# dvalcarce/filmyou-core

Hardware: AMD Instinct MI355X
Metric: top-N recs/sec (RM2), ml25m shape (higher is better)
Workload: dtype f32 (scores and logs fp32 / v_log_f32, folded in fp64; co-rating sums 64-bit fixed point in LDS (fp64 fallback); G stored as 24-bit e7m17 floats scaled per cluster above 4096 items; ratings fp16 in the row kernel when exactly representable)

## Files before the change

### filmyou-core_amd/_native.py

```python
import ctypes as C
import os
import subprocess

_HERE = os.path.dirname(os.path.abspath(__file__))
CSRC = os.path.join(_HERE, "csrc")
LIB_DIR = os.path.join(_HERE, "lib")
LIB_PATH = os.path.join(LIB_DIR, "libfilmyou_hip.so")
INCLUDE = os.path.join(os.path.dirname(_HERE), "include", "filmyou.h")
SOURCES = ["fy_api.hip", "fy_prep.hip", "fy_rm2.hip", "fy_rm2_request.hip", "fy_rm1.hip", "fy_ratings_update.hip", "fy_itemsim.hip", "fy_itemsim_request.hip", "fy_itemcf.hip", "fy_itemcf_request.hip", "fy_itemcf_estimate.hip", "fy_eval.hip", "fy_cluster.hip", "fy_nmf.hip", "fy_refine.hip", "fy_rccl.hip", "fy_seqfile.cpp"]
HEADERS = ["fy_common.hpp", "fy_tuning.hpp", "fy_rm2_plan.hpp", "fy_rm2_tables.hpp", "fy_partition.hpp", "fy_prep.hpp", "fy_cooc.hpp", "fy_cooc_tables.hpp", "fy_rm2.hpp", "fy_rm2_kernels.hpp", "fy_rm2_launch.hpp", "fy_rm2_coop.hpp", "fy_rm2_request.hpp", "fy_rm1.hpp", "fy_ratings_update.hpp", "fy_refine.hpp", "fy_itemsim_plan.hpp", "fy_itemsim_kernels.hpp", "fy_itemsim_request.hpp", "fy_itemcf_request.hpp", "fy_eval.hpp"]
HIPCC_FLAGS = ["--offload-arch=gfx950", "-O3", "-std=c++17", "-fPIC", "-shared", "-munsafe-fp-atomics", "-Wall",
               "-Wno-unused-result", "-ldl"]

SYMBOLS = [
    "fy_abi_version", "fy_last_error", "fy_context_create", "fy_context_destroy", "fy_context_synchronize", "fy_context_reload_tuning", "fy_context_inject_alloc_failure",
    "fy_context_stream", "fy_ratings_create", "fy_ratings_destroy", "fy_ratings_nnz", "fy_ratings_drop_cache", "fy_ratings_apply", "fy_ratings_copy_out", "fy_rm2_prepare",
    "fy_rm2_partial_stats", "fy_rm2_stats_layout", "fy_rm2_set_global_stats", "fy_rm2_set_collectives", "fy_rccl_unique_id", "fy_rccl_create", "fy_rccl_collectives", "fy_rccl_counters", "fy_rccl_destroy", "fy_rccl_detach_context", "fy_rm2_score", "fy_rm2_score_users", "fy_result_request_stats", "fy_rm2_job_destroy", "fy_rm2_run",
    "fy_itemsim_build", "fy_itemsim_run", "fy_itemsim_prepare", "fy_itemsim_job_destroy", "fy_itemsim_rows", "fy_result_itemsim_request_stats", "fy_itemcf_recommend", "fy_itemcf_recommend_filtered", "fy_itemcf_recommend_prepared", "fy_result_itemcf_request_stats", "fy_itemsim_job_drop_rows", "fy_ratings_shifted", "fy_itemsim_pairs",
    "fy_simpairs_write_text", "fy_idfile_read", "fy_cluster_assign", "fy_nmf_factorize", "fy_result_size", "fy_result_key0", "fy_result_key1", "fy_result_value",
    "fy_result_aux", "fy_result_n_users", "fy_result_user_id", "fy_result_user_sum", "fy_result_n_items",
    "fy_result_item_id", "fy_result_item_coll", "fy_result_total_sum", "fy_result_free", "fy_result_stats",
    "fy_seqfile_read_int_int", "fy_seqfile_read_int_double", "fy_seqfile_read_intpair_float", "fy_seqfile_write_int_int",
    "fy_seqfile_write_int_double", "fy_seqfile_write_intpair_float", "fy_mapfile_write_int_double", "fy_buffer_free",
    "fy_submap_create", "fy_submap_n_users", "fy_submap_n_items", "fy_submap_nnz", "fy_submap_counts", "fy_submap_users",
    "fy_submap_items", "fy_submap_matrix", "fy_submap_destroy", "fy_cluster_refine", "fy_refined_n_users", "fy_refined_n_counts",
    "fy_refined_clustering", "fy_refined_layout", "fy_refined_h_size", "fy_refined_w_size", "fy_refined_factors",
    "fy_refined_stats", "fy_refined_free",
    "fy_ratings_holdout", "fy_result_create_lists", "fy_eval_prepare", "fy_eval_lists", "fy_eval_destroy",
    "fy_itemcf_estimate_prepared", "fy_itemcf_estimate_ratings", "fy_result_itemcf_estimate_stats", "fy_eval_estimates",
]


def _stale():
    if not os.path.exists(LIB_PATH):
        return True
    t = os.path.getmtime(LIB_PATH)
    deps = [os.path.join(CSRC, f) for f in SOURCES + HEADERS] + [INCLUDE]
    return any(os.path.getmtime(d) > t for d in deps)


def build(force=False, verbose=False):
    if not force and not _stale():
        build_host_driver()
        return LIB_PATH
    from concurrent.futures import ThreadPoolExecutor
    obj_dir = os.path.join(LIB_DIR, "obj")
    os.makedirs(obj_dir, exist_ok=True)
    hipcc = os.environ.get("HIPCC", "/opt/rocm/bin/hipcc")
    if not os.path.exists(hipcc):
        hipcc = "hipcc"
    cflags = [f for f in HIPCC_FLAGS if f not in ("-shared", "-ldl")]
    common = max(os.path.getmtime(d) for d in [os.path.join(CSRC, h) for h in HEADERS] + [INCLUDE])
    import hashlib
    stamp_path = os.path.join(obj_dir, "flags.stamp")
    stamp = hashlib.sha256(("\0".join([os.path.realpath(hipcc)] + cflags)).encode()).hexdigest()
    try:
        with open(stamp_path) as f:
            same_flags = f.read().strip() == stamp
    except OSError:
        same_flags = False
    if not same_flags:
        force = True

    def compile_one(src):
        path, obj = os.path.join(CSRC, src), os.path.join(obj_dir, src + ".o")
        if not force and os.path.exists(obj) and os.path.getmtime(obj) > max(common, os.path.getmtime(path)):
            return obj
        cmd = [hipcc] + cflags + ["-c", "-o", obj, path]
        if verbose:
            print(" ".join(cmd))
        subprocess.run(cmd, check=True)
        return obj

    with ThreadPoolExecutor(max_workers=min(len(SOURCES), os.cpu_count() or 1)) as ex:
        objs = list(ex.map(compile_one, SOURCES))
    with open(stamp_path, "w") as f:
        f.write(stamp + "\n")
    cmd = [hipcc, "--offload-arch=gfx950", "-fPIC", "-shared", "-o", LIB_PATH] + objs + ["-ldl"]
    if verbose:
        print(" ".join(cmd))
    subprocess.run(cmd, check=True)
    build_host_driver()
    return LIB_PATH


HOST_DIR = os.path.join(_HERE, "host")
HOST_DRIVER = os.path.join(HOST_DIR, "rm2_main")


def build_host_driver():
    src = os.path.join(HOST_DIR, "rm2_main.cpp")
    hdr = os.path.join(HOST_DIR, "filmyou_job.hpp")
    if os.path.exists(HOST_DRIVER) and all(os.path.getmtime(HOST_DRIVER) >= os.path.getmtime(p) for p in (src, hdr, LIB_PATH)):
        return HOST_DRIVER
    subprocess.run(["g++", "-std=c++17", "-O2", "-Wall", "-o", HOST_DRIVER, src, "-L" + LIB_DIR, "-lfilmyou_hip",
                    "-Wl,-rpath,$ORIGIN/../lib"], check=True)
    return HOST_DRIVER


class RM2Params(C.Structure):
    _fields_ = [("lambda_", C.c_double), ("number_of_items", C.c_int32), ("number_of_recommendations", C.c_int32),
                ("filter_users", C.c_int32), ("number_of_clusters", C.c_int32), ("rank", C.c_int32),
                ("world", C.c_int32), ("flags", C.c_uint32), ("workspace_bytes", C.c_int64)]


ALL_GATHER_FN = C.CFUNCTYPE(C.c_int, C.c_void_p, C.c_void_p, C.c_void_p, C.c_int64, C.c_void_p)
REDUCE_SCATTER_FN = C.CFUNCTYPE(C.c_int, C.c_void_p, C.c_void_p, C.c_void_p, C.c_int64, C.c_void_p)


class Collectives(C.Structure):
    _fields_ = [("user", C.c_void_p), ("all_gather", ALL_GATHER_FN), ("reduce_scatter_f32", REDUCE_SCATTER_FN)]


class NMFParams(C.Structure):
    _fields_ = [("number_of_users", C.c_int32), ("number_of_items", C.c_int32), ("number_of_clusters", C.c_int32),
                ("number_of_iterations", C.c_int32), ("ppc", C.c_int32), ("normalization_frequency", C.c_int32)]


class RefineParams(C.Structure):
    _fields_ = [("number_of_users", C.c_int32), ("number_of_clusters", C.c_int32), ("users_per_sub_cluster", C.c_int32),
                ("number_of_iterations", C.c_int32), ("ppc", C.c_int32), ("normalization_frequency", C.c_int32),
                ("seed", C.c_uint64)]


class RefineStats(C.Structure):
    _fields_ = [("ms_mappings", C.c_double), ("ms_iterations", C.c_double), ("ms_assign", C.c_double), ("ms_total", C.c_double),
                ("launches", C.c_int64), ("sum_users", C.c_int64), ("sum_items", C.c_int64), ("sum_k", C.c_int64),
                ("nnz", C.c_int64), ("collisions", C.c_int64)]

    def as_dict(self):
        return {k: getattr(self, k) for k, _ in self._fields_}


class ItemSimParams(C.Structure):
    _fields_ = [("similarity", C.c_int32), ("max_similarities_per_item", C.c_int32), ("exclude_self", C.c_int32),
                ("has_threshold", C.c_int32), ("threshold", C.c_double), ("rank", C.c_int32), ("world", C.c_int32),
                ("flags", C.c_uint32), ("min_prefs_per_user", C.c_int32), ("max_prefs_per_user", C.c_int32)]


class ItemCFParams(C.Structure):
    _fields_ = [("num_recommendations", C.c_int32), ("max_prefs_per_user", C.c_int32), ("boolean_data", C.c_int32),
                ("rank", C.c_int32), ("world", C.c_int32), ("flags", C.c_uint32)]


class ItemCFFilter(C.Structure):
    _fields_ = [("has_users", C.c_int32), ("has_items", C.c_int32), ("n_users", C.c_int64), ("users", C.c_void_p),
                ("n_items", C.c_int64), ("items", C.c_void_p)]


class RM2Request(C.Structure):
    _fields_ = [("n_users", C.c_int64), ("users", C.c_void_p)]


class RM2RequestStats(C.Structure):
    _fields_ = [("users_asked", C.c_int64), ("users_known", C.c_int64), ("clusters_touched", C.c_int64), ("batches", C.c_int64),
                ("slab_rows", C.c_int64), ("slab_bytes_peak", C.c_int64), ("slab_pair_contribs", C.c_int64),
                ("full_pass_clusters", C.c_int64)]

    def as_dict(self):
        return {k: getattr(self, k) for k, _ in self._fields_}


class ItemSimRequest(C.Structure):
# ... 205 lines not shown
```

### filmyou-core_amd/csrc/fy_api.hip

```cpp
#include <algorithm>
#include <cstdlib>
#include <memory>
#include <mutex>
#include <new>
#include <unordered_map>

#include "fy_prep.hpp"
#include "fy_rm2.hpp"
#include "fy_ratings_update.hpp"
#include "fy_rm2_request.hpp"
#include "fy_itemsim_request.hpp"
#include "fy_itemcf_request.hpp"
#include "fy_eval.hpp"

namespace fy {
static thread_local char g_err[512] = "";
void set_error(const char* fmt, ...) {
    va_list ap;
    va_start(ap, fmt);
    vsnprintf(g_err, sizeof g_err, fmt, ap);
    va_end(ap);
}
const char* last_error() { return g_err; }
}

using namespace fy;

void fy::load_tuning_from_env(Tuning& t) {
    t = Tuning{};
    if (const char* e = getenv("FY_M24")) t.pack24 = atoi(e) != 0;
    if (const char* e = getenv("FY_M24_MIN_ITEMS")) t.pack24_min_items = std::max(0, atoi(e));
    if (const char* e = getenv("FY_SCORE_SLICES")) t.max_slices = atoi(e);
    if (const char* e = getenv("FY_SCORE_UPW")) { int v = atoi(e); if (v >= 1) t.users_per_wave = v; }
    if (const char* e = getenv("FY_PRUNE")) t.prune = atoi(e) != 0;
    if (const char* e = getenv("FY_LAZY_MIRROR")) t.lazy_mirror = atoi(e) != 0;
    if (const char* e = getenv("FY_REFINE")) t.refine = atoi(e) != 0;
    if (const char* e = getenv("FY_REFINE_C")) { double v = atof(e); if (v >= 0.0 && v < 1e6) t.refine_c = (float)v; }
    if (const char* e = getenv("FY_FULL_WALK_SPARSE")) t.full_walk_sparse = atoi(e) != 0;
    if (const char* e = getenv("FY_PREP_PACKED")) t.prep_packed = atoi(e) != 0;
    if (const char* e = getenv("FY_OVERLAP_VALUES")) t.overlap_values = atoi(e) != 0;
    if (const char* e = getenv("FY_SHARD_PREP")) t.shard_prep = atoi(e) != 0;
    if (const char* e = getenv("FY_SUP_BOUNDS")) t.sup_bounds = atoi(e) != 0;
    if (const char* e = getenv("FY_COOP")) t.coop = atoi(e) != 0;
    if (const char* e = getenv("FY_COOP_FORCE")) t.coop_force = atoi(e) != 0;
    if (const char* e = getenv("FY_COOC_PK")) t.cooc_pk = atoi(e) != 0;
    if (const char* e = getenv("FY_COOC_F32")) t.cooc_f32 = atoi(e) != 0;
    if (const char* e = getenv("FY_COOC_HALF")) t.cooc_half = atoi(e) != 0;
    if (const char* e = getenv("FY_COOC_RECT")) t.cooc_rect = atoi(e) != 0;
    if (const char* e = getenv("FY_COOC_FX")) t.cooc_fx = atoi(e) != 0;
    if (const char* e = getenv("FY_PANEL_MIN_CLUSTERS")) { int v = atoi(e); if (v >= 1) t.panel_min_clusters = v; }
    if (const char* e = getenv("FY_PANEL_COLS")) { int v = atoi(e); if (v >= 256) { t.panel_cols = v; t.panel_wide_below_users = 0; } }
    if (const char* e = getenv("FY_PANEL_WIDE_BELOW_USERS")) { int v = atoi(e); if (v >= 0) t.panel_wide_below_users = v; }
    if (const char* e = getenv("FY_PANEL_MAX_CH")) { int v = atoi(e); if (v >= 256) t.panel_max_ch = v; }
    if (const char* e = getenv("FY_COOC_PLANES")) t.cooc_planes = atoi(e) != 0;
    if (const char* e = getenv("FY_SCORE_HEAVY")) { int v = atoi(e); if (v >= 0) t.score_heavy = v; }
    if (const char* e = getenv("FY_SCORE_WALK")) t.score_walk = atoi(e) != 0;
    if (const char* e = getenv("FY_COOC_EPI")) t.cooc_epi = atoi(e) != 0;
    if (const char* e = getenv("FY_TOPN_SEED_XL")) t.topn_seed_xl = atoi(e) != 0;
    if (const char* e = getenv("FY_PANEL_REPAIR")) t.panel_repair = atoi(e) != 0;
    if (const char* e = getenv("FY_PANEL_MULTI_LAUNCH")) t.panel_multi_launch = atoi(e) != 0;
    if (const char* e = getenv("FY_FLAT")) t.flat_batch = atoi(e) != 0;
    if (const char* e = getenv("FY_PANEL_SYM")) t.panel_sym = atoi(e) != 0;
    if (const char* e = getenv("FY_DEBUG_SYNC")) t.debug_sync = atoi(e);
    if (const char* e = getenv("FY_PANEL_GROUP_MB")) t.panel_group_bytes = std::max<int64_t>(0, (int64_t)atoll(e)) << 20;
    if (const char* e = getenv("FY_FLAT_BUDGET_MB")) t.flat_budget = std::max<int64_t>(0, (int64_t)atoll(e)) << 20;
    if (const char* e = getenv("FY_PANEL_TWO_PHASE")) t.panel_two_phase = atoi(e) != 0;
    if (const char* e = getenv("FY_PANEL_LANES")) { int v = atoi(e); if (v >= 1 && v <= 8) t.panel_lanes = v; }
    if (const char* e = getenv("FY_PRUNE_MIN_ITEMS")) { t.prune_min_items = atoi(e); t.prune_min_users = 0; }
    if (const char* e = getenv("FY_PRUNE_MIN_USERS")) { int v = atoi(e); if (v >= 0) t.prune_min_users = v; }
    if (const char* e = getenv("FY_SEED_CHUNKS")) { int v = atoi(e); if (v >= 0 && v <= 40) { t.seed_chunks = v; t.seed_forced = v > 0; } }
    if (const char* e = getenv("FY_WORKSPACE_GB")) { long v = atol(e); if (v >= 1) t.workspace_default = (int64_t)v << 30; }
    if (const char* e = getenv("FY_LANES")) { int v = atoi(e); if (v >= 1 && v <= 8) { t.lanes = v; t.lanes_forced = true; } }
    if (const char* e = getenv("FY_COOC_BLOCK")) { int v = atoi(e); if (v == 256 || v == 512 || v == 1024) t.cooc_block = v; }
    if (const char* e = getenv("FY_COOC_MAX_CH")) { int v = atoi(e); if (v >= 64 && v <= 20224) { t.cooc_max_ch = v; t.cooc_max_ch_forced = true; } }
    if (const char* e = getenv("FY_TOPN_FORCE_SELECT")) t.force_select = atoi(e) != 0;
    if (const char* e = getenv("FY_MAX_SURV_FRAC")) { double v = atof(e); if (v >= 0.0) t.max_surv_frac = v; }
    if (const char* e = getenv("FY_REQ_FULL_SHARE")) { double v = atof(e); if (v >= 0.0) t.req_full_share = v; }
    if (const char* e = getenv("FY_REQ_CHUNK")) { int v = atoi(e); if (v >= 64 && v <= 16384 && v % 64 == 0) t.req_chunk = v; }
    if (const char* e = getenv("FY_RM1_NBR_CHUNK")) { int v = atoi(e); if (v >= 1 && v <= (1 << 20)) t.rm1_nbr_chunk = v; }
    if (const char* e = getenv("FY_RM1_COL_CHUNK")) { int v = atoi(e); if (v >= 1 && v <= (1 << 20)) t.rm1_col_chunk = v; }
    if (const char* e = getenv("FY_UPD_LDS_KEYS")) { int v = atoi(e); if (v >= 0 && v <= fy::UPD_LDS_KEYS_MAX) t.upd_lds_keys = v; }
    if (const char* e = getenv("FY_ISIM_HEAVY")) t.isim_heavy = std::max(0, atoi(e));
    if (const char* e = getenv("FY_ISIM_GRAM")) t.isim_gram = atoi(e) != 0;
    if (const char* e = getenv("FY_ISIM_GRAM_MIN_ITEMS")) t.isim_gram_min_items = std::max(0, atoi(e));
    if (const char* e = getenv("FY_ISIM_CAPG")) { int v = atoi(e); if (v >= 1 && v <= 2040) t.isim_capg = v; }
    if (const char* e = getenv("FY_ISIM_ACC32")) t.isim_acc32 = atoi(e) != 0;
    if (const char* e = getenv("FY_ISIM_PIECE")) { int v = atoi(e); if (v >= 64 && v <= 8192 && v % 64 == 0) t.isim_piece = v; }
    if (const char* e = getenv("FY_ISIM_REQ_CHUNK")) { int v = atoi(e); if (v >= 64 && v <= 16384 && v % 64 == 0) t.isim_req_chunk = v; }
    if (const char* e = getenv("FY_ISIM_REQ_ROWS")) t.isim_req_rows = std::max(0, atoi(e));
    if (const char* e = getenv("FY_ICF_EST_CHUNK")) { int v = atoi(e); if (v >= 1 && v <= fy::ICF_EST_CHUNK_MAX) t.icf_est_chunk = v; }
}

namespace {
std::mutex& g_jobs_mu = *new std::mutex;
std::unordered_map<const fy_rm2_job*, fy::Context*>& g_jobs = *new std::unordered_map<const fy_rm2_job*, fy::Context*>;
fy::Context* job_context(const fy_rm2_job* j) {
    std::lock_guard<std::mutex> g(g_jobs_mu);
    auto it = g_jobs.find(j);
    return it == g_jobs.end() ? nullptr : it->second;
}
inline void select_device(const fy::Context* ctx) {
    if (ctx) FY_HIP(hipSetDevice(ctx->device));
}
}

#define FY_TRY try {
#define FY_CATCH                                                           \
    }                                                                      \
    catch (const fy::Failure& f) { return f.code; }                        \
    catch (const std::bad_alloc&) {                                        \
        fy::set_error("host allocation failed");                           \
        return FY_ERR_OUT_OF_MEMORY;                                       \
    }                                                                      \
    catch (const std::exception& e) {                                      \
        fy::set_error("unexpected: %s", e.what());                         \
        return FY_ERR_HIP;                                                 \
    }                                                                      \
    return FY_OK;

extern "C" {

int fy_abi_version(void) { return FY_ABI_VERSION; }
const char* fy_last_error(void) { return fy::last_error(); }

int fy_context_create(int device_ordinal, fy_context** out) {
    if (!out) { set_error("out is NULL"); return FY_ERR_INVALID_ARGUMENT; }
    *out = nullptr;
    FY_TRY
    int n = 0;
    hipError_t e = hipGetDeviceCount(&n);
    if (e != hipSuccess || n <= 0) {
        (void)hipGetLastError();
        FY_FAIL(FY_ERR_NO_DEVICE, "no HIP device is visible (%s); this library has no CPU fallback",
                e == hipSuccess ? "device count 0" : hipGetErrorString(e));
    }
    if (device_ordinal < 0 || device_ordinal >= n) FY_FAIL(FY_ERR_INVALID_ARGUMENT, "device %d of %d", device_ordinal, n);
    FY_HIP(hipSetDevice(device_ordinal));
    hipDeviceProp_t prop;
    FY_HIP(hipGetDeviceProperties(&prop, device_ordinal));
    if (std::string(prop.gcnArchName).rfind("gfx950", 0) != 0)
        FY_FAIL(FY_ERR_NO_DEVICE, "device %d is %s; the kernels are built for gfx950 (MI355X) only", device_ordinal, prop.gcnArchName);
    std::unique_ptr<fy_context> c(new fy_context);
    c->c.device = device_ordinal;
    c->c.num_cus = prop.multiProcessorCount;
    c->c.total_mem = prop.totalGlobalMem;
    FY_HIP(hipStreamCreateWithFlags(&c->c.stream, hipStreamNonBlocking));
    fy::load_tuning_from_env(c->c.tune);
    *out = c.release();
    FY_CATCH
}

void fy_context_destroy(fy_context* c) {
    if (!c) return;
    (void)hipSetDevice(c->c.device);
    if (c->c.stream) {
        for (hipStream_t x : c->c.aux) (void)hipStreamSynchronize(x);
        (void)hipStreamSynchronize(c->c.stream);
        c->c.trim();
        for (auto& kv : c->c.capacity) (void)hipFree(kv.first);
        c->c.capacity.clear();
        for (hipStream_t x : c->c.aux) { (void)hipStreamSynchronize(x); (void)hipStreamDestroy(x); }
        (void)hipStreamDestroy(c->c.stream);
    }
    delete c;
}

int fy_context_inject_alloc_failure(fy_context* c, int64_t nth) {
    if (!c || nth < 0) { set_error("context is NULL or nth < 0"); return FY_ERR_INVALID_ARGUMENT; }
    c->c.fail_alloc_in = nth;
    return FY_OK;
}

int fy_context_reload_tuning(fy_context* c) {
    if (!c) { set_error("context is NULL"); return FY_ERR_INVALID_ARGUMENT; }
    fy::load_tuning_from_env(c->c.tune);
    return FY_OK;
}

int fy_context_synchronize(fy_context* c) {
    if (!c) { set_error("context is NULL"); return FY_ERR_INVALID_ARGUMENT; }
    FY_TRY
    select_device(&c->c);
    FY_HIP(hipStreamSynchronize(c->c.stream));
    FY_CATCH
}

void* fy_context_stream(fy_context* c) { return c ? (void*)c->c.stream : nullptr; }

int fy_ratings_create(fy_context* c, int64_t nnz, const int32_t* user, const int32_t* item, const float* score, int location,
                      fy_ratings** out) {
    if (!out) { set_error("out is NULL"); return FY_ERR_INVALID_ARGUMENT; }
    *out = nullptr;
    if (!c) { set_error("context is NULL"); return FY_ERR_INVALID_ARGUMENT; }
    if (nnz < 0 || (nnz > 0 && (!user || !item || !score))) { set_error("ratings arrays are NULL or nnz < 0"); return FY_ERR_INVALID_ARGUMENT; }
    if (location != FY_HOST && location != FY_DEVICE) { set_error("location must be FY_HOST or FY_DEVICE"); return FY_ERR_INVALID_ARGUMENT; }
    FY_TRY
    FY_HIP(hipSetDevice(c->c.device));
    std::unique_ptr<fy_ratings> r(new fy_ratings);
    r->ctx = &c->c;
    r->nnz = nnz;
    r->user.alloc(&c->c, (size_t)nnz);
    r->item.alloc(&c->c, (size_t)nnz);
    r->score.alloc(&c->c, (size_t)nnz);
    if (nnz) {
        const hipMemcpyKind k = location == FY_HOST ? hipMemcpyHostToDevice : hipMemcpyDeviceToDevice;
        FY_HIP(hipMemcpyAsync(r->user.get(), user, (size_t)nnz * 4, k, c->c.stream));
        FY_HIP(hipMemcpyAsync(r->item.get(), item, (size_t)nnz * 4, k, c->c.stream));
        FY_HIP(hipMemcpyAsync(r->score.get(), score, (size_t)nnz * 4, k, c->c.stream));
        FY_HIP(hipStreamSynchronize(c->c.stream));
        fy::ratings_id_bounds(&c->c, r.get());
// ... 465 lines not shown
```

### filmyou-core_amd/csrc/fy_cooc.hpp

```cpp
#pragma once
#include <hip/hip_fp16.h>

#include <type_traits>

#include "fy_common.hpp"
#include "fy_prep.hpp"
#include "fy_rm2_plan.hpp"
#include "fy_rm2_tables.hpp"

namespace fy {

struct CoocArgs {
    const int32_t* __restrict__ rank_pair;
    const int32_t* __restrict__ pair_start;
    const int32_t* __restrict__ seg_ptr;
    const int2* __restrict__ seg;
    const float* __restrict__ seg_w;
    const int32_t* __restrict__ csr_idx;
    const float* __restrict__ csr_w;
    int32_t pbase;
    int32_t slot_base;
    int32_t Ic;
    int32_t CH;
    int32_t nch;
    int32_t row0;
    int32_t nrows;
    int32_t q0;
    int32_t nq;
    const int32_t* __restrict__ local_start;
    int32_t row_stride;
    const uint32_t* __restrict__ csr_pk;
    const int2* __restrict__ item_seg;
    uint32_t pk_bytes;
    const int32_t* __restrict__ item_id;
    int32_t half;
    double fx_scale;
    int32_t tail_row0, tail_chunks;
    int32_t item_grab;
    int32_t acc_quarter;
    int32_t acc32;
    int32_t half_rows, head_chunks;
};
__device__ __forceinline__ bool cooc_row_is_cut(const CoocArgs& A, int row) { return A.half && (A.half_rows == 0 || row < A.half_rows); }
__device__ __forceinline__ int cooc_acc_index(int c, int quarter) { return quarter ? (c & 3) * quarter + (c >> 2) : c; }

#ifndef FY_COOC_NB
#define FY_COOC_NB 8
#endif
extern __shared__ __attribute__((aligned(16))) double fy_cooc_acc[];

struct SegBatch {
    int2 d;
    float w;
};
static_assert(FY_COOC_NB == 8, "the segment groups of cooc_seg_slot are 8 segments long");
__device__ __forceinline__ int cooc_seg_slot(int s_begin, int batch, int wave, int nwaves, int lane) {
    return s_begin + ((((batch << 3) + (lane >> 3)) * nwaves + wave) << 3) + (lane & 7);
}
__device__ __forceinline__ SegBatch cooc_first_batch(const CoocArgs& A, int s_begin, int s_end) {
    const int lane = threadIdx.x & 63;
    const int wave = __builtin_amdgcn_readfirstlane(threadIdx.x >> 6);
    SegBatch B{make_int2(0, 0), 0.0f};
    const int s = cooc_seg_slot(s_begin, 0, wave, blockDim.x >> 6, lane);
    if (s < s_end) { B.d = A.seg[s]; B.w = A.seg_w[s]; }
    return B;
}

template <bool PK, class ACC>
__device__ __forceinline__ void cooc_accumulate_segments(const CoocArgs& A, ACC* __restrict__ acc, int s_begin, int s_end, int c0, SegBatch first,
                                                         int rmask = -1 ) {
    const int lane = threadIdx.x & 63;
    const int wave = __builtin_amdgcn_readfirstlane(threadIdx.x >> 6);
    const int nwaves = blockDim.x >> 6;
    const int32_t* __restrict__ csr_idx = A.csr_idx;
    const float* __restrict__ csr_w = A.csr_w;
    const uint32_t* __restrict__ csr_pk = A.csr_pk;
    constexpr int NB = FY_COOC_NB;
    struct Group {
        int L[NB];
        float W[NB];
        int idx[NB];
        float x[NB];
    };
    auto issue = [&](Group& G, const int2& d, float w, int g) __attribute__((always_inline)) {
#pragma unroll
        for (int q = 0; q < NB; q++) {
            const int F = __builtin_amdgcn_readlane(d.x, g + q);
            G.L[q] = __builtin_amdgcn_readlane(d.y, g + q);
            G.W[q] = __uint_as_float(__builtin_amdgcn_readlane(__float_as_uint(w), g + q));
            const int at = F + (lane < G.L[q] ? lane : 0);
            G.x[q] = 0.0f;
            if constexpr (PK) G.idx[q] = (int)csr_pk[at];
            else {
                G.idx[q] = csr_idx[at] - c0;
                G.x[q] = csr_w[at];
            }
        }
    };
    auto commit = [&](Group& G) __attribute__((always_inline)) {
        if constexpr (PK) {
#pragma unroll
            for (int q = 0; q < NB; q++) {
                const uint32_t pk = (uint32_t)G.idx[q];
                G.x[q] = __half2float(__ushort_as_half((unsigned short)(pk >> 16)));
                G.idx[q] = (int)(pk & 0xFFFFu);
            }
        }
#pragma unroll
        for (int q = 0; q < NB; q++)
            if (lane < G.L[q] && G.idx[q] > rmask) atomicAdd(&acc[cooc_acc_index(G.idx[q], A.acc_quarter)], (ACC)G.W[q] * (ACC)G.x[q]);
    };
    int batch = 0;
    if (cooc_seg_slot(s_begin, 0, wave, nwaves, 0) >= s_end) return;
    int2 d = first.d;
    float w = first.w;
    while (true) {
        const int nloc = __popcll(__ballot(cooc_seg_slot(s_begin, batch, wave, nwaves, lane) < s_end));
        const int s_next = cooc_seg_slot(s_begin, batch + 1, wave, nwaves, lane);
        int2 dn = make_int2(0, 0);
        float wn = 0.0f;
        if (s_next < s_end) { dn = A.seg[s_next]; wn = A.seg_w[s_next]; }
        Group GA, GB;
        issue(GA, d, w, 0);
#pragma unroll 1
        for (int g = 0; g < 64; g += 2 * NB) {
            issue(GB, d, w, g + NB);
            commit(GA);
            if (g + 2 * NB < 64) issue(GA, d, w, g + 2 * NB);
            commit(GB);
            if (g + 2 * NB >= nloc) break;
        }
        d = dn;
        w = wn;
        batch++;
        if (cooc_seg_slot(s_begin, batch, wave, nwaves, 0) >= s_end) break;
    }
}

struct PkGroup {
    int L[FY_COOC_NB];
    float W[FY_COOC_NB];
    uint32_t pk[FY_COOC_NB];
};
__device__ __forceinline__ void cooc_pk_issue(const __amdgpu_buffer_rsrc_t rsrc, int lane4, PkGroup& G, const int2& d, float w, int g) {
#pragma unroll
    for (int q = 0; q < FY_COOC_NB; q++) {
        const int F = __builtin_amdgcn_readlane(d.x, g + q);
        G.L[q] = __builtin_amdgcn_readlane(d.y, g + q);
        G.W[q] = __uint_as_float(__builtin_amdgcn_readlane(__float_as_uint(w), g + q));
        G.pk[q] = (uint32_t)__builtin_amdgcn_raw_buffer_load_b32(rsrc, lane4, F * 4, 0);
    }
}
__device__ __forceinline__ __amdgpu_buffer_rsrc_t cooc_pk_rsrc(const CoocArgs& A) {
    return __builtin_amdgcn_make_buffer_rsrc(const_cast<uint32_t*>(A.csr_pk), 0, (int)A.pk_bytes, 0x00020000);
}
template <class ACC>
__device__ __forceinline__ void cooc_accumulate_pk(const CoocArgs& A, ACC* __restrict__ acc, int s_begin, int s_end, SegBatch first,
                                                   int rmask = -1 ) {
    const int lane = threadIdx.x & 63;
    const int wave = __builtin_amdgcn_readfirstlane(threadIdx.x >> 6);
    const int nwaves = blockDim.x >> 6;
    const __amdgpu_buffer_rsrc_t rsrc = cooc_pk_rsrc(A);
    const int lane4 = lane * 4;
    constexpr int NB = FY_COOC_NB;
    using Group = PkGroup;
    auto issue = [&](Group& G, const int2& d, float w, int g) __attribute__((always_inline)) { cooc_pk_issue(rsrc, lane4, G, d, w, g); };
    const double fx = A.fx_scale;
    const uint32_t ix_mask = A.acc_quarter ? 3u : 0u, ix_shift = A.acc_quarter ? 2u : 0u, ix_quarter = (uint32_t)A.acc_quarter;
    auto commit = [&](Group& G) __attribute__((always_inline)) {
#pragma unroll
        for (int q = 0; q < NB; q++) {
            const float x = __half2float(__ushort_as_half((unsigned short)(G.pk[q] >> 16)));
            if constexpr (std::is_same<ACC, uint32_t>::value) {
                const uint32_t v = (uint32_t)(G.W[q] * x * (float)fx);
                if (lane < G.L[q] && (int)(G.pk[q] & 0xFFFFu) > rmask) atomicAdd(&acc[cooc_acc_index((int)(G.pk[q] & 0xFFFFu), A.acc_quarter)], v);
            } else if constexpr (std::is_same<ACC, unsigned long long>::value) {
                const double d = fma((double)(G.W[q] * x), fx, 4503599627370496.0);
                unsigned long long v = (unsigned long long)__double_as_longlong(d) & 0xFFFFFFFFFFFFFull;
                const uint32_t c = G.pk[q] & 0xFFFFu;
                uint32_t at = __umul24(c & ix_mask, ix_quarter) + (c >> ix_shift);
                asm volatile("" : "+v"(at), "+v"(v));
                if (lane < G.L[q] && (int)c > rmask) atomicAdd(&acc[at], v);
            } else {
                const ACC v = (ACC)(G.W[q] * x);
                if (lane < G.L[q] && (int)(G.pk[q] & 0xFFFFu) > rmask) atomicAdd(&acc[cooc_acc_index((int)(G.pk[q] & 0xFFFFu), A.acc_quarter)], v);
            }
        }
    };
    int batch = 0;
    if (cooc_seg_slot(s_begin, 0, wave, nwaves, 0) >= s_end) return;
    int2 d = first.d;
    float w = first.w;
    while (true) {
        const int nloc = __popcll(__ballot(cooc_seg_slot(s_begin, batch, wave, nwaves, lane) < s_end));
        const int s_next = cooc_seg_slot(s_begin, batch + 1, wave, nwaves, lane);
        int2 dn = make_int2(0, 0);
        float wn = 0.0f;
        if (s_next < s_end) { dn = A.seg[s_next]; wn = A.seg_w[s_next]; }
        Group GA, GB;
        issue(GA, d, w, 0);
#pragma unroll 1
        for (int g = 0; g < 64; g += 2 * NB) {
            issue(GB, d, w, g + NB);
            commit(GA);
            if (g + 2 * NB < 64) issue(GA, d, w, g + 2 * NB);
            commit(GB);
            if (g + 2 * NB >= nloc) break;
        }
        d = dn;
        w = wn;
        batch++;
        if (cooc_seg_slot(s_begin, batch, wave, nwaves, 0) >= s_end) break;
    }
}

template <bool PK = false>
__device__ __forceinline__ void cooc_accumulate_row(const CoocArgs& A, int row, int ch, int lrow = 0) {
    int s_begin, s_end;
    if (A.item_seg) {
        const int2 se = A.item_seg[(int64_t)lrow * A.nch + ch];
        s_begin = se.x;
        s_end = se.y;
    } else {
        const int pair = A.rank_pair[A.pbase + row];
        int e0 = A.pair_start[pair], e1 = A.pair_start[pair + 1];
        if (A.local_start) { e0 = A.local_start[lrow]; e1 = A.local_start[lrow + 1]; }
        const int32_t* __restrict__ sp = A.seg_ptr + (int64_t)ch * (A.nq + 1) - A.q0;
        s_begin = sp[e0];
        s_end = sp[e1];
    }
    if constexpr (PK) cooc_accumulate_pk<double>(A, fy_cooc_acc, s_begin, s_end, cooc_first_batch(A, s_begin, s_end));
    else cooc_accumulate_segments<false, double>(A, fy_cooc_acc, s_begin, s_end, ch * A.CH, cooc_first_batch(A, s_begin, s_end));
}

__attribute__((unused)) static __global__ void k_item_segments(CoocArgs A, int2* __restrict__ out) {
    const int n = A.nrows * A.nch;
    const int stride = A.row_stride ? A.row_stride : 1;
    for (int t = blockIdx.x * blockDim.x + threadIdx.x; t < n; t += gridDim.x * blockDim.x) {
        const int lrow = t / A.nch, ch = t % A.nch;
        const int pair = A.rank_pair[A.pbase + A.row0 + lrow * stride];
        int e0 = A.pair_start[pair], e1 = A.pair_start[pair + 1];
        if (A.local_start) { e0 = A.local_start[lrow]; e1 = A.local_start[lrow + 1]; }
        const int32_t* __restrict__ sp = A.seg_ptr + (int64_t)ch * (A.nq + 1) - A.q0;
        out[t] = make_int2(sp[e0], sp[e1]);
    }
}

__host__ __device__ inline int64_t cooc_half_item_index(int32_t row, int32_t ch, int32_t CH, int32_t nch) {
    const int64_t c = row / CH;
    return (int64_t)CH * (c * nch - c * (c - 1) / 2) + (int64_t)(row - c * CH) * (nch - c) + (ch - c);
}
__host__ __device__ inline int64_t cooc_rect_item_index(int32_t row, int32_t ch, int32_t CH) {
    const int64_t c = row / CH;
    return (int64_t)CH * (c * (c + 1) / 2) + (int64_t)(row - c * CH) * (c + 1) + ch;
}
__host__ __device__ inline bool cooc_tile_stored(int B, int T, int bpc) {
    if (bpc <= 0) return T > B;
    const int cB = B / bpc, cT = T / bpc;
    return cT == cB ? T > B : cT < cB;
}
inline int64_t cooc_item_count(int32_t nrows, int32_t CH, int32_t nch, int half) {
    if (!half) return (int64_t)nrows * nch;
    if (half == 2) return nrows > 0 ? cooc_rect_item_index(nrows - 1, (nrows - 1) / CH, CH) + 1 : 0;
    return nrows > 0 ? cooc_half_item_index(nrows - 1, nch - 1, CH, nch) + 1 : 0;
}
__device__ __forceinline__ void item_list_body(const CoocArgs& A, int2* __restrict__ seg_out, int32_t* __restrict__ id_out) {
    const int n = A.nrows * A.nch;
    const int stride = A.row_stride ? A.row_stride : 1;
    for (int t = blockIdx.x * blockDim.x + threadIdx.x; t < n; t += gridDim.x * blockDim.x) {
        const int lrow = t / A.nch, ch = t % A.nch;
        const int row = A.row0 + lrow * stride;
        int64_t at = t;
        if (A.half && A.half_rows > 0) {
            if (row < A.half_rows) {
                if (ch < row / A.CH || ch >= A.head_chunks) continue;
                at = cooc_half_item_index(row, ch, A.CH, A.head_chunks);
            } else {
                if (ch >= A.tail_chunks) continue;
                at = cooc_half_item_index(A.half_rows - 1, A.head_chunks - 1, A.CH, A.head_chunks) + 1 + (int64_t)(row - A.half_rows) * A.tail_chunks + ch;
            }
        } else if (A.half == 2) {
            if (ch > row / A.CH) continue;
            at = cooc_rect_item_index(row, ch, A.CH);
        } else if (A.half) {
            if (ch < row / A.CH) continue;
            at = cooc_half_item_index(row, ch, A.CH, A.nch);
        } else if (A.tail_chunks > 0 && lrow >= A.tail_row0) {
            if (ch >= A.tail_chunks) continue;
            at = (int64_t)A.tail_row0 * A.nch + (int64_t)(lrow - A.tail_row0) * A.tail_chunks + ch;
        }
        const int pair = A.rank_pair[A.pbase + row];
        int e0 = A.pair_start[pair], e1 = A.pair_start[pair + 1];
        if (A.local_start) { e0 = A.local_start[lrow]; e1 = A.local_start[lrow + 1]; }
        const int32_t* __restrict__ sp = A.seg_ptr + (int64_t)ch * (A.nq + 1) - A.q0;
        seg_out[at] = make_int2(sp[e0], sp[e1]);
        id_out[at] = (lrow << 8) | ch;
    }
}
__attribute__((unused)) static __global__ void k_item_list(CoocArgs A, int2* __restrict__ seg_out, int32_t* __restrict__ id_out) {
    item_list_body(A, seg_out, id_out);
}

struct SegTable {
    const int32_t* ptr = nullptr;
    const int2* seg = nullptr;
    const float* w = nullptr;
};
struct CoocGeometry {
    int32_t pbase, slot_base;
    int32_t Ic, CH, nch;
    int32_t q0, nq;
};
inline CoocGeometry cooc_geometry(const Plan& p) { return CoocGeometry{p.pbase, p.sbase, p.Ic, p.CH, p.nch, p.q0, p.nq}; }
inline CoocArgs cooc_args(const Prepared& P, const SegTable& T, const CoocGeometry& g, const float* csr_w, const uint32_t* csr_pk) {
    CoocArgs A{};
    A.rank_pair = P.rank_pair.get(); A.pair_start = P.pair_start.get(); A.seg_ptr = T.ptr; A.seg = T.seg; A.seg_w = T.w;
    A.csr_idx = P.csr_idx.get(); A.csr_w = csr_w; A.csr_pk = csr_pk; A.pk_bytes = (uint32_t)std::min<int64_t>((int64_t)P.nnz * 4, 0xFFFFFFFFll);
    A.pbase = g.pbase; A.slot_base = g.slot_base; A.Ic = g.Ic; A.CH = g.CH; A.nch = g.nch; A.nrows = g.Ic; A.q0 = g.q0; A.nq = g.nq;
    return A;
}
struct SegArrays {
    const int32_t* __restrict__ csc_slot;
    const float* __restrict__ csc_w;
    const int32_t* __restrict__ chunk_off;
    const int32_t* __restrict__ row_of_entry;
    const int32_t* __restrict__ samples;
};
struct SegGroup {
    SegArrays in;
    const SegDesc* desc;
    size_t n;
};
struct SegStore {
    int64_t n_seg = 0;
    DevBuf<int32_t> ptr;
    DevBuf<int2> seg;
    DevBuf<float> w;
    SegTable view(const SegDesc& d) const { return SegTable{ptr.get() + d.cnt_off, seg.get(), w.get()}; }
};
void build_segment_tables(Context* ctx, const SegGroup* groups, size_t n_groups, SegStore& out, hipStream_t st = nullptr);
inline void build_segment_table(Context* ctx, const SegArrays& in, const SegDesc& d, SegStore& out, hipStream_t st = nullptr) {
    const SegGroup g{in, &d, 1};
    build_segment_tables(ctx, &g, 1, out, st);
}
void build_csr_samples(Context* ctx, int64_t nnz, const int32_t* csr_idx, DevBuf<int32_t>& samp, hipStream_t st = nullptr);

struct CsrDescs {
    std::vector<CsrDesc> h;
    DevBuf<CsrDesc> d;
};
CsrDescs upload_csr_descs(Context* ctx, std::vector<CsrDesc> h, hipStream_t st = nullptr);
void build_chunk_offsets(Context* ctx, const CsrDescs& C, const int32_t* rowptr, const int32_t* csr_idx, int32_t* co_all, hipStream_t st = nullptr);
void pack_csr(Context* ctx, const CsrDescs& C, const int32_t* csr_idx, const float* csr_r, uint32_t* pk, hipStream_t st = nullptr);

__host__ __device__ inline int cooc_lds_columns(int CH) { return (CH % 256 == 0) ? CH : ((CH + 255) / 256) * 256 + 256; }


}
```

### filmyou-core_amd/csrc/fy_rm2.hip

```cpp
#include <algorithm>
#include <cmath>
#include <cstdlib>
#include <type_traits>

#include "fy_cooc.hpp"
#include "fy_prep.hpp"
#include <chrono>
#include "fy_rm2.hpp"
#include "fy_rm2_plan.hpp"
#include "fy_rm1.hpp"
#include "fy_rm2_request.hpp"

namespace fy {

constexpr int PAIR_HEAVY = 2048;
struct PairPass {
    const int32_t* __restrict__ rank_pair;
    const int32_t* __restrict__ pair_start;
    const int32_t* __restrict__ pair_di;
    const int32_t* __restrict__ csc_slot;
    const float* __restrict__ csc_r;
    const double2* __restrict__ ud_slot;
    int32_t lo, hi;
    float* __restrict__ csc_x;
// ... 270 lines not shown
        const double p = icoll[pair_di[rank_pair[pos]]];
        p_rank[pos] = p;
        pb_rank[pos] = make_double2(p, b_rank[pos]);
        if constexpr (GEN) a_rank[pos] = (float)p;
        else a_rank[pos] = (float)(lambda * p);
        b_rank32[pos] = (float)b_rank[pos];
    }
}

__global__ void k_csc_x(int64_t nnz, const int32_t* __restrict__ csc_slot, const float* __restrict__ csc_r,
                        const double* __restrict__ usum_slot, float* __restrict__ csc_x, float* __restrict__ csc_x_over_s) {
    for (int64_t q = blockIdx.x * (int64_t)blockDim.x + threadIdx.x; q < nnz; q += (int64_t)gridDim.x * blockDim.x) {
        const double s = usum_slot[csc_slot[q]];
        const double x = (double)csc_r[q] / s;
        csc_x[q] = (float)x;
        if (csc_x_over_s) csc_x_over_s[q] = (float)(x / s);
    }
}

__global__ void k_csc_rank(int64_t nnz, const int32_t* __restrict__ csc_pair, const int32_t* __restrict__ pair_rank, int32_t* __restrict__ out) {
    for (int64_t q = blockIdx.x * (int64_t)blockDim.x + threadIdx.x; q < nnz; q += (int64_t)gridDim.x * blockDim.x) out[q] = pair_rank[csc_pair[q]];
}

#include "fy_cooc_tables.hpp"

template <bool GEN>
__global__ void k_csr_values(int32_t nU, const int32_t* __restrict__ rowptr, const int32_t* __restrict__ csr_idx,
                             const float* __restrict__ csr_r, const int32_t* __restrict__ slot2du,
                             const int32_t* __restrict__ ucluster, const double* __restrict__ usum,
                             const int32_t* __restrict__ csize, const int32_t* __restrict__ pcstart,
                             const double2* __restrict__ pb_rank, double lambda,
                             const float* __restrict__ gscale ,
                             float* __restrict__ csr_x, float* __restrict__ csr_e, float* __restrict__ csr_q,
                             const double* __restrict__ usum_slot, SmoothArgs G) {
    const int lane = threadIdx.x & 63;
    const int wpb = blockDim.x >> 6;
    for (int32_t s = blockIdx.x * wpb + (threadIdx.x >> 6); s < nU; s += gridDim.x * wpb) {
        const int32_t du = slot2du[s];
        const int32_t c = ucluster[du];
        const double sum = GEN ? usum_slot[s] : usum[du];
        const double Uc1 = (double)(csize[c] - 1);
        const double gs = (double)gscale[c];
        const int32_t pb = pcstart[c];
        for (int32_t f = rowptr[s] + lane; f < rowptr[s + 1]; f += 64) {
            const int32_t j = csr_idx[f];
            const double x = (double)csr_r[f] / sum;
            const double2 pbj = pb_rank[pb + j];
            if constexpr (GEN) {
                const double e = fy_e_general(pbj.y, pbj.x, (double)csr_r[f], sum, (double)G.deg_slot[s], G.beta_slot[s], G.s2_cluster[c], G.bt_scale, G.bt_by_n);
                csr_x[f] = (float)x;
                csr_e[f] = (float)(e * gs);
                csr_q[f] = (float)(pbj.x * gs);
                continue;
            }
            double e = (1.0 - lambda) * (pbj.y - x) + lambda * Uc1 * pbj.x;
            if (!(e > 0.0)) e = 0.0;
            csr_x[f] = (float)x;
            csr_e[f] = (float)(e * gs);
            csr_q[f] = (float)(lambda * (1.0 - lambda) * pbj.x * gs);
        }
    }
}

__global__ void k_user_meta(int32_t lo, int32_t hi, const int32_t* __restrict__ slot2du, const int32_t* __restrict__ uid,
                            const int32_t* __restrict__ ucluster, const int32_t* __restrict__ udeg,
                            const int32_t* __restrict__ csize, const int32_t* __restrict__ pcstart, int32_t number_of_items,
                            int32_t top_n, int32_t filter_users, const int32_t* __restrict__ cshift ,
                            double* __restrict__ pvpi, int32_t* __restrict__ n_out,
                            unsigned long long* __restrict__ counters ) {
    unsigned long long terms = 0, scored = 0;
    for (int32_t s = lo + blockIdx.x * blockDim.x + threadIdx.x; s < hi; s += gridDim.x * blockDim.x) {
        const int32_t du = slot2du[s];
        const int32_t c = ucluster[du];
        const int32_t n = udeg[du];
        const int32_t Ic = pcstart[c + 1] - pcstart[c];
        const int32_t unrated = Ic - n;
        pvpi[s - lo] = (double)(n - 1) * log((double)number_of_items) - (double)n * log((double)csize[c]) +
                       (double)n * (double)cshift[c] * 0.69314718055994530942;
        const bool skip = unrated <= 0 || uid[du] < filter_users;
        int32_t k = skip ? 0 : min(top_n, unrated);
        if (k < 0) k = 0;
        n_out[s - lo] = k;
        if (!skip) { terms += (unsigned long long)n * (unsigned long long)unrated; scored++; }
    }
    for (int o = 32; o > 0; o >>= 1) {
        terms += __shfl_down(terms, o, 64);
        scored += __shfl_down(scored, o, 64);
    }
    if ((threadIdx.x & 63) == 0) {
        if (terms) atomicAdd(&counters[0], terms);
        if (scored) atomicAdd(&counters[1], scored);
    }
}

constexpr int FY_P24_SHIFT = 6;
struct MEpilogue {
    float* __restrict__ M;
    int64_t ldm;
    float w2;
    double fx_inv;
    int pack24;
    float* __restrict__ Bmax;
    int64_t ldb;
    int local_rows;
    int32_t panel_cols;
    float* __restrict__ Bmax64;
    int64_t ldb64;
    uint32_t* __restrict__ Brep;
    int64_t pitch;
    int ceil24;
    double* __restrict__ head32;
    int64_t ld_head;
    int32_t head_rows;
    double* __restrict__ tail32;
    int32_t tail_from;
    double w2d;
};

#define FY_ROR16(x, n) ((uint32_t)__builtin_amdgcn_update_dpp(0, (int)(x), 0x120 + (n), 0xF, 0xF, false))
__device__ __forceinline__ uint32_t fy_max_half_wave(uint32_t m) {
    m = max(m, FY_ROR16(m, 8));
    m = max(m, FY_ROR16(m, 4));
    m = max(m, FY_ROR16(m, 2));
    m = max(m, FY_ROR16(m, 1));
    const auto r = __builtin_amdgcn_permlane16_swap(m, m, false, false);
    return max((uint32_t)r[0], (uint32_t)r[1]);
}
__device__ __forceinline__ uint32_t fy_max_wave(uint32_t m) {
    m = fy_max_half_wave(m);
    const auto r = __builtin_amdgcn_permlane32_swap(m, m, false, false);
    return max((uint32_t)r[0], (uint32_t)r[1]);
}

template <class ACC, int EPI>
__device__ __forceinline__ bool cooc_epilogue_takes_eight(const CoocArgs& A, const MEpilogue& E) {
    return EPI && sizeof(ACC) == 8 && A.acc_quarter && !(A.acc_quarter & 1) && !E.Bmax64 && !E.panel_cols && !E.pitch;
}
template <class ACC>
__device__ __forceinline__ void cooc_rm2_tail_copy(const CoocArgs& A, const MEpilogue& E, const ACC* __restrict__ acc, int row, int c0, int c_end) {
    double* __restrict__ tp = E.tail32 + (int64_t)(row - E.tail_from) * E.head_rows;
    for (int col = c0 + (int)(threadIdx.x >> 6) * 512 + (int)(threadIdx.x & 63) * 8; col < c_end; col += (int)blockDim.x * 8) {
        double t[8];
#pragma unroll
        for (int k = 0; k < 8; k++) {
            const ACC a = acc[cooc_acc_index(col - c0 + k, A.acc_quarter)];
            if constexpr (std::is_integral<ACC>::value) t[k] = (double)a * E.fx_inv;
            else t[k] = E.w2d * (double)a;
        }
        double2* __restrict__ o = reinterpret_cast<double2*>(tp + col);
#pragma unroll
        for (int k = 0; k < 4; k++) o[k] = make_double2(t[2 * k], t[2 * k + 1]);
    }
}
template <class ACC, bool COPY, int EPI>
__device__ __forceinline__ void cooc_rm2_epilogue_pack(const CoocArgs& A, const MEpilogue& E, ACC* __restrict__ acc, int row, int mrow, int c0, int c1, int cb,
                                                       int first_bmax_block) {
        const int64_t row_cols = E.pitch ? E.pitch : (E.panel_cols ? E.panel_cols : E.ldm);
        const uint32_t radd = E.ceil24 ? (1u << FY_P24_SHIFT) - 1u : 1u << (FY_P24_SHIFT - 1);
        if constexpr (EPI && !COPY && sizeof(ACC) == 8) {
        if (A.acc_quarter && !(A.acc_quarter & 1) && !E.Bmax64 && !E.panel_cols && !E.pitch) {
            using Pair = typename std::conditional<std::is_integral<ACC>::value, uint4, double2>::type;
            const int qz = A.acc_quarter;
            char* __restrict__ out = reinterpret_cast<char*>(E.M) + (int64_t)mrow * E.ldm * 3;
            const int l8 = (int)(threadIdx.x & 63) * 8, step = (int)blockDim.x * 8;
            int cw = cb + __builtin_amdgcn_readfirstlane((int)(threadIdx.x >> 6)) * 512;
            auto fetch = [&](int col, Pair* p) __attribute__((always_inline)) {
                const Pair* ap = reinterpret_cast<const Pair*>(acc + ((min(col, c1 - 8) - c0) >> 2));
#pragma unroll
                for (int q = 0; q < 4; q++) p[q] = ap[(q * qz) >> 1];
            };
            auto trip = [&](int col, const Pair* p) __attribute__((always_inline)) {
                const bool on = col < c1;
                if (on) {
                    Pair* ap = reinterpret_cast<Pair*>(acc + ((col - c0) >> 2));
#pragma unroll
                    for (int q = 0; q < 4; q++) ap[(q * qz) >> 1] = Pair{};
                }
                uint32_t v[8];
#pragma unroll
                for (int q = 0; q < 4; q++) {
#pragma unroll
                    for (int h = 0; h < 2; h++) {
                        float f;
                        if constexpr (std::is_integral<ACC>::value) {
                            const double d = __builtin_fma((double)(h ? p[q].w : p[q].y), 4294967296.0, (double)(h ? p[q].z : p[q].x));
                            f = (float)(d * E.fx_inv);
                        } else f = E.w2 * (float)(h ? p[q].y : p[q].x);
                        v[4 * h + q] = (__float_as_uint(f) + radd) >> FY_P24_SHIFT;
                    }
                }
                if (on) {
                    uint32_t* __restrict__ o = reinterpret_cast<uint32_t*>(out + (int64_t)col * 3);
                    o[0] = v[0] | (v[1] << 24);
                    o[1] = (v[1] >> 8) | (v[2] << 16);
                    o[2] = (v[2] >> 16) | (v[3] << 8);
                    o[3] = v[4] | (v[5] << 24);
                    o[4] = (v[5] >> 8) | (v[6] << 16);
                    o[5] = (v[6] >> 16) | (v[7] << 8);
                }
                if (E.Bmax) {
                    uint32_t m = max(max(max(v[0], v[1]), max(v[2], v[3])), max(max(v[4], v[5]), max(v[6], v[7])));
                    m = fy_max_half_wave(on ? m : 0u);
                    if ((threadIdx.x & 31) == 0 && m && (col >> 8) >= first_bmax_block) {
                        uint8_t* bp = reinterpret_cast<uint8_t*>(E.Bmax) + ((int64_t)mrow * E.ldb + (col >> 8)) * 3;
                        bp[0] = (uint8_t)m;
                        bp[1] = (uint8_t)(m >> 8);
                        bp[2] = (uint8_t)(m >> 16);
                    }
                }
            };
            Pair pa[4], pb[4];
            if (cw < c1) fetch(cw + l8, pa);
            while (cw < c1) {
                if (cw + step < c1) fetch(cw + step + l8, pb);
                trip(cw + l8, pa);
                cw += step;
                if (cw >= c1) break;
                if (cw + step < c1) fetch(cw + step + l8, pa);
                trip(cw + l8, pb);
                cw += step;
            }
            return;
        }
        }
        uint32_t* __restrict__ out3 = reinterpret_cast<uint32_t*>(reinterpret_cast<char*>(E.M) + (int64_t)mrow * row_cols * 3);
        for (int c4 = (cb >> 2) + threadIdx.x; 4 * c4 < c1; c4 += blockDim.x) {
            uint32_t v[4];
            const int qz = A.acc_quarter;
            ACC* ap = acc + (qz ? c4 - (c0 >> 2) : 4 * c4 - c0);
            const int qs = qz ? qz : 1;
            double f4[COPY ? 4 : 1];
#pragma unroll
            for (int q = 0; q < 4; q++) {
                float f;
                if constexpr (std::is_integral<ACC>::value) { const double d = (double)ap[q * qs] * E.fx_inv; f = (float)d; if constexpr (COPY) f4[q] = d; }
                else { f = E.w2 * (float)ap[q * qs]; if constexpr (COPY) f4[q] = E.w2d * (double)ap[q * qs]; }
                ap[q * qs] = (ACC)0;
                v[q] = (__float_as_uint(f) + radd) >> FY_P24_SHIFT;
            }
            if constexpr (COPY) {
            if (E.head32 && mrow < E.head_rows && 4 * c4 < E.ld_head) {
                double2* hp = reinterpret_cast<double2*>(E.head32 + (int64_t)mrow * E.ld_head + 4 * c4);
                hp[0] = make_double2(f4[0], f4[1]);
                hp[1] = make_double2(f4[2], f4[3]);
            }
            if (E.tail32 && row >= E.tail_from && 4 * c4 < E.head_rows) {
                double2* tp = reinterpret_cast<double2*>(E.tail32 + (int64_t)(row - E.tail_from) * E.head_rows + 4 * c4);
                tp[0] = make_double2(f4[0], f4[1]);
                tp[1] = make_double2(f4[2], f4[3]);
            }
            }
            if (!E.panel_cols || 4 * c4 < E.panel_cols) {
                out3[3 * c4 + 0] = v[0] | (v[1] << 24);
                out3[3 * c4 + 1] = (v[1] >> 8) | (v[2] << 16);
                out3[3 * c4 + 2] = (v[2] >> 16) | (v[3] << 8);
            }
            if (E.Bmax64) {
                const uint32_t cq = (uint32_t)((4 * c4) & 63);
                const uint32_t k0 = (v[0] << 6) | cq, k1 = (v[1] << 6) | (cq + 1), k2 = (v[2] << 6) | (cq + 2), k3 = (v[3] << 6) | (cq + 3);
                const uint32_t a1 = max(k0, k1), a2 = min(k0, k1), b1 = max(k2, k3), b2 = min(k2, k3);
                uint32_t t1 = max(a1, b1), t2 = max(min(a1, b1), max(a2, b2));
#define FY_TOP2_STEP(n)                                         \
    {                                                           \
        const uint32_t p1 = FY_ROR16(t1, n), p2 = FY_ROR16(t2, n); \
        t2 = max(min(t1, p1), max(t2, p2));                     \
        t1 = max(t1, p1);                                       \
    }
                FY_TOP2_STEP(8) FY_TOP2_STEP(4) FY_TOP2_STEP(2) FY_TOP2_STEP(1)
#undef FY_TOP2_STEP
                const uint32_t m = t1 >> 6;
                if ((threadIdx.x & 15) == 0 && m) {
                    uint8_t* bp = reinterpret_cast<uint8_t*>(E.Bmax64) + ((int64_t)mrow * E.ldb64 + (c4 >> 4)) * 3;
                    bp[0] = (uint8_t)m;
                    bp[1] = (uint8_t)(m >> 8);
                    bp[2] = (uint8_t)(m >> 16);
                    if (E.Brep) E.Brep[(int64_t)mrow * E.ldb64 + (c4 >> 4)] = ((t2 >> 6) << 8) | (t1 & 63u);
                }
            }
            if (E.Bmax) {
                uint32_t m = max(max(v[0], v[1]), max(v[2], v[3]));
                if constexpr (EPI) m = fy_max_wave(m);
                else {
#pragma unroll
                    for (int o = 1; o < 64; o <<= 1) m = max(m, (uint32_t)__shfl_xor((int)m, o, 64));
                }
                if ((threadIdx.x & 63) == 0 && m && (c4 >> 6) >= first_bmax_block) {
                    uint8_t* bp = reinterpret_cast<uint8_t*>(E.Bmax) + ((int64_t)mrow * E.ldb + (c4 >> 6)) * 3;
                    bp[0] = (uint8_t)m;
                    bp[1] = (uint8_t)(m >> 8);
                    bp[2] = (uint8_t)(m >> 16);
                }
            }
        }
}

template <class ACC, int EPI>
__device__ __forceinline__ void cooc_rm2_epilogue(const CoocArgs& A, const MEpilogue& E, ACC* __restrict__ acc, int id) {
    const int lrow = id >> 8;
    const int row = A.row0 + lrow * (A.row_stride ? A.row_stride : 1);
    const int mrow = E.local_rows ? lrow : row;
    const int ch = id & 255;
    const int c0 = ch * A.CH;
    const int c1 = (ch == A.nch - 1) ? (int)E.ldm : min(c0 + A.CH, (int)E.ldm);
    const bool front = A.half == 2 && c0 + A.CH <= row;
    const int cb = (cooc_row_is_cut(A, row) && c0 <= row && !front) ? (row & ~255) : c0;
    const int first_bmax_block = (A.half && !front) ? (row >> 8) + 1 : 0;
    if (E.pack24) {
        const bool tail_item = E.tail32 && row >= E.tail_from && c0 < E.head_rows && (A.half != 2 || front);
        const bool tail8 = tail_item && A.half == 2 && cooc_epilogue_takes_eight<ACC, EPI>(A, E);
        const bool copy = E.head32 && (mrow < E.head_rows || (tail_item && !tail8));
        if (copy) cooc_rm2_epilogue_pack<ACC, true, EPI>(A, E, acc, row, mrow, c0, c1, cb, first_bmax_block);
        else {
            if (tail8) cooc_rm2_tail_copy<ACC>(A, E, acc, row, c0, min(c1, (int)E.head_rows));
            cooc_rm2_epilogue_pack<ACC, false, EPI>(A, E, acc, row, mrow, c0, c1, cb, first_bmax_block);
        }
    } else {
        float* __restrict__ out = E.M + (int64_t)mrow * E.ldm;
        for (int col = cb + threadIdx.x; col < c1; col += blockDim.x) {
            const int at = cooc_acc_index(col - c0, A.acc_quarter);
            if constexpr (std::is_integral<ACC>::value) out[col] = (float)((double)acc[at] * E.fx_inv);
            else out[col] = E.w2 * (float)acc[at];
            acc[at] = (ACC)0;
        }
    }
}

template <bool PK, class ACC, int EPI>
__device__ __forceinline__ void cooc_rm2_body(const CoocArgs& A, const MEpilogue& E, int n_items, int* __restrict__ next_item) {
    ACC* __restrict__ acc = reinterpret_cast<ACC*>(fy_cooc_acc);
    __shared__ int sh_item, sh_s0, sh_s1, sh_id;
    const int CHp = cooc_lds_columns(A.CH);
    for (int t = threadIdx.x; t < CHp; t += blockDim.x) acc[t] = (ACC)0;
    const int ITEM_GRAB = A.item_grab > 0 ? A.item_grab : 1;
    int next = 0, next2 = 0;
    int g_cur = 0, g_end = 0, g_next = 0;
    auto grab = [&]() __attribute__((always_inline)) {
        if (g_cur == g_end) {
            g_cur = g_next;
            g_end = g_cur + ITEM_GRAB;
            g_next = atomicAdd(next_item, ITEM_GRAB);
        }
        return g_cur++;
    };
    if (threadIdx.x == 0) {
        g_cur = atomicAdd(next_item, ITEM_GRAB);
        g_end = g_cur + ITEM_GRAB;
        g_next = atomicAdd(next_item, ITEM_GRAB);
        const int first = grab();
        next = grab();
        const int2 se = first < n_items ? A.item_seg[first] : make_int2(0, 0);
        sh_item = first;
        sh_s0 = se.x;
        sh_s1 = se.y;
        sh_id = first < n_items ? A.item_id[first] : 0;
    }
    __syncthreads();
    int item = sh_item, s0 = sh_s0, s1 = sh_s1, id = sh_id;
    __syncthreads();
    SegBatch batch = cooc_first_batch(A, s0, s1);
    while (item < n_items) {
        int2 se_next = make_int2(0, 0);
        int id_next = 0;
        if (threadIdx.x == 0) {
            next2 = grab();
            if (next < n_items) { se_next = A.item_seg[next]; id_next = A.item_id[next]; }
        }
        const int c0 = (id & 255) * A.CH;
        const int row_of_item = A.row0 + (id >> 8) * (A.row_stride ? A.row_stride : 1);
        const int rmask = (cooc_row_is_cut(A, row_of_item) && row_of_item >= c0 && row_of_item < c0 + A.CH) ? row_of_item - c0 : -1;
        if constexpr (PK) cooc_accumulate_pk<ACC>(A, acc, s0, s1, batch, rmask);
        else cooc_accumulate_segments<false, ACC>(A, acc, s0, s1, c0, batch, rmask);
        if (threadIdx.x == 0) { sh_item = next; sh_s0 = se_next.x; sh_s1 = se_next.y; sh_id = id_next; }
        __syncthreads();
        const int nitem = sh_item;
        s0 = sh_s0;
        s1 = sh_s1;
        const int nid = sh_id;
        batch = cooc_first_batch(A, s0, s1);
        cooc_rm2_epilogue<ACC, EPI>(A, E, acc, id);
        item = nitem;
        id = nid;
        if (threadIdx.x == 0) next = next2;
        __syncthreads();
    }
}
template <bool PK, class ACC, int ROLE = 0, int EPI = 1>
__global__ void k_cooc_rm2(CoocArgs A, MEpilogue E, int n_items, int* __restrict__ next_item) {
    cooc_rm2_body<PK, ACC, EPI>(A, E, n_items, next_item);
}
struct CoocLaunch {
    CoocArgs A;
    MEpilogue E;
    int32_t n_items, pad;
};
template <bool PK, class ACC, int ROLE = 0, int EPI = 1>
__global__ void k_cooc_rm2_multi(const CoocLaunch* __restrict__ D, int* __restrict__ counters) {
    const CoocLaunch& d = D[blockIdx.y];
    const CoocArgs A = d.A;
    const MEpilogue E = d.E;
    cooc_rm2_body<PK, ACC, EPI>(A, E, d.n_items, counters + blockIdx.y);
}
__global__ void k_item_list_multi(const CoocLaunch* __restrict__ D) {
    const CoocArgs A = D[blockIdx.y].A;
    item_list_body(A, const_cast<int2*>(A.item_seg), const_cast<int32_t*>(A.item_id));
}

__device__ __forceinline__ void fy_unpack24_raw(uint32_t d0, uint32_t d1, uint32_t d2, uint32_t* v) {
    v[0] = d0 & 0xFFFFFFu;
    v[1] = (d0 >> 24) | ((d1 & 0xFFFFu) << 8);
    v[2] = (d1 >> 16) | ((d2 & 0xFFu) << 16);
    v[3] = d2 >> 8;
}
__device__ __forceinline__ uint32_t fy_load24(const uint32_t* __restrict__ row3, int e) {
    const int g = e >> 2;
    uint32_t v[4];
    fy_unpack24_raw(row3[3 * g], row3[3 * g + 1], row3[3 * g + 2], v);
    return v[e & 3];
}
constexpr int MIRROR_PITCH = 772;

extern __shared__ __attribute__((aligned(16))) unsigned char fy_mirror_lds[];
__device__ __forceinline__ void mirror_tiles_body(float* __restrict__ M_, int64_t ldm, int32_t Ic, float* __restrict__ Bmax_, int64_t ldb,
                                                  const int32_t* __restrict__ need = nullptr, int32_t write_below = 0x7FFFFFFF,
                                                  int32_t bpc = 0 ) {
    __shared__ uint32_t rowmax[128];
    const int tj = blockIdx.x, B = blockIdx.y;
    if ((tj >> 1) == B || !cooc_tile_stored(B, tj >> 1, bpc)) return;
    const int dst_row0 = 128 * tj;
    if (dst_row0 >= Ic) return;
    const bool write = B < write_below || (need && need[B] != 0);
    if (!write && !Bmax_) return;
    const int lane = threadIdx.x & 63, wave = threadIdx.x >> 6, nwaves = blockDim.x >> 6;
    const int64_t pitch = ldm * 3;
    unsigned char* __restrict__ Mb = reinterpret_cast<unsigned char*>(M_);
    if (threadIdx.x < 128) rowmax[threadIdx.x] = 0;
    __syncthreads();
    const int m = lane & 31, h = lane >> 5;
    uint32_t mx[4] = {0, 0, 0, 0};
    for (int r = 2 * wave + h; r < 256; r += 2 * nwaves) {
        const int src_row = 256 * B + r;
        uint32_t v[4] = {0, 0, 0, 0};
        if (src_row < Ic) {
            const uint32_t* __restrict__ p = reinterpret_cast<const uint32_t*>(Mb + (int64_t)src_row * pitch + (int64_t)dst_row0 * 3) + 3 * m;
            fy_unpack24_raw(p[0], p[1], p[2], v);
        }
#pragma unroll
        for (int q = 0; q < 4; q++) {
            if (write) {
                unsigned char* d = fy_mirror_lds + (4 * m + q) * MIRROR_PITCH + 3 * r;
                d[0] = (unsigned char)v[q];
                d[1] = (unsigned char)(v[q] >> 8);
                d[2] = (unsigned char)(v[q] >> 16);
            }
            mx[q] = max(mx[q], v[q]);
        }
    }
#pragma unroll
    for (int q = 0; q < 4; q++)
        if (mx[q]) atomicMax(&rowmax[4 * m + q], mx[q]);
    __syncthreads();
    for (int c = wave; write && c < 128; c += nwaves) {
        const int dst_row = dst_row0 + c;
        if (dst_row >= Ic) break;
        const uint32_t* __restrict__ sp = reinterpret_cast<const uint32_t*>(fy_mirror_lds + c * MIRROR_PITCH) + 3 * lane;
        uint32_t* __restrict__ dp = reinterpret_cast<uint32_t*>(Mb + (int64_t)dst_row * pitch + (int64_t)256 * B * 3) + 3 * lane;
        dp[0] = sp[0];
        dp[1] = sp[1];
        dp[2] = sp[2];
    }
    if (Bmax_ && threadIdx.x < 128 && dst_row0 + (int)threadIdx.x < Ic) {
        const uint32_t pv = rowmax[threadIdx.x];
        uint8_t* bp = reinterpret_cast<uint8_t*>(Bmax_) + ((int64_t)(dst_row0 + threadIdx.x) * ldb + B) * 3;
        bp[0] = (uint8_t)pv;
        bp[1] = (uint8_t)(pv >> 8);
        bp[2] = (uint8_t)(pv >> 16);
    }
}

__global__ __launch_bounds__(1024) void k_mirror_tiles(float* __restrict__ M_, int64_t ldm, int32_t Ic, float* __restrict__ Bmax_, int64_t ldb,
                                                       const int32_t* __restrict__ need, int32_t write_below, int32_t bpc) {
    mirror_tiles_body(M_, ldm, Ic, Bmax_, ldb, need, write_below, bpc);
}
__global__ __launch_bounds__(1024) void k_colmax_upper(const float* __restrict__ M_, int64_t ldm, int32_t Ic, float* __restrict__ Bmax_, int64_t ldb, int32_t first_block,
                                                       int32_t bpc) {
    __shared__ uint32_t colmax[256];
    const int tj = blockIdx.x, B = first_block + blockIdx.y;
    if (tj == B || !cooc_tile_stored(B, tj, bpc) || 256 * B >= Ic) return;
    const int col0 = 256 * tj;
    if (col0 >= Ic) return;
    const int lane = threadIdx.x & 63, wave = threadIdx.x >> 6;
    const int64_t pitch = ldm * 3;
    const unsigned char* __restrict__ Mb = reinterpret_cast<const unsigned char*>(M_);
    if (threadIdx.x < 256) colmax[threadIdx.x] = 0;
    __syncthreads();
    uint32_t mx[4] = {0, 0, 0, 0};
    const int r_end = min(256, Ic - 256 * B);
    uint32_t d[4][3];
#pragma unroll
    for (int step = 0; step < 4; step++) {
#pragma unroll
        for (int x = 0; x < 4; x++) {
            const int r = wave * 16 + step * 4 + x;
            const uint32_t* __restrict__ p = reinterpret_cast<const uint32_t*>(Mb + (int64_t)(256 * B + min(r, r_end - 1)) * pitch + (int64_t)col0 * 3) + 3 * lane;
            d[x][0] = p[0]; d[x][1] = p[1]; d[x][2] = p[2];
        }
#pragma unroll
        for (int x = 0; x < 4; x++) {
            uint32_t v[4];
            fy_unpack24_raw(d[x][0], d[x][1], d[x][2], v);
#pragma unroll
            for (int q = 0; q < 4; q++) mx[q] = max(mx[q], v[q]);
        }
    }
#pragma unroll
    for (int q = 0; q < 4; q++)
        if (mx[q]) atomicMax(&colmax[4 * lane + q], mx[q]);
    __syncthreads();
    if (threadIdx.x < 256 && col0 + (int)threadIdx.x < Ic) {
        const uint32_t pv = colmax[threadIdx.x];
        uint8_t* bp = reinterpret_cast<uint8_t*>(Bmax_) + ((int64_t)(col0 + threadIdx.x) * ldb + B) * 3;
        bp[0] = (uint8_t)pv;
        bp[1] = (uint8_t)(pv >> 8);
        bp[2] = (uint8_t)(pv >> 16);
    }
}
__global__ void k_flag_surviving_blocks(int32_t n_users, const int32_t* __restrict__ n_quads, const uint16_t* __restrict__ surv, int64_t ldb, int32_t* __restrict__ need) {
    for (int32_t u = blockIdx.x; u < n_users; u += gridDim.x)
        for (int k = threadIdx.x; k < n_quads[u]; k += blockDim.x) {
            const int b = surv[(int64_t)u * ldb + k];
            if (need[b] == 0) need[b] = 1;
        }
}
__device__ __forceinline__ void mirror_diag_body(float* __restrict__ M_, int64_t ldm, int32_t Ic, float* __restrict__ Bmax_, int64_t ldb) {
    const int B = blockIdx.x, c = threadIdx.x;
    const int row = 256 * B + c;
    if (row >= Ic) return;
    const int64_t pitch = ldm * 3;
    unsigned char* __restrict__ Mb = reinterpret_cast<unsigned char*>(M_);
    uint32_t* __restrict__ own = reinterpret_cast<uint32_t*>(Mb + (int64_t)row * pitch + (int64_t)256 * B * 3);
    uint32_t best = 0;
    for (int g = 0; g < 64; g++) {
        uint32_t v[4];
        if (4 * g >= c) {
            fy_unpack24_raw(own[3 * g], own[3 * g + 1], own[3 * g + 2], v);
        } else {
            if (4 * g + 3 >= c) fy_unpack24_raw(own[3 * g], own[3 * g + 1], own[3 * g + 2], v);
#pragma unroll
            for (int q = 0; q < 4; q++) {
                const int r = 4 * g + q;
                if (r < c) v[q] = fy_load24(reinterpret_cast<const uint32_t*>(Mb + (int64_t)(256 * B + r) * pitch + (int64_t)256 * B * 3), c);
            }
            own[3 * g + 0] = v[0] | (v[1] << 24);
            own[3 * g + 1] = (v[1] >> 8) | (v[2] << 16);
            own[3 * g + 2] = (v[2] >> 16) | (v[3] << 8);
        }
        best = max(max(best, max(v[0], v[1])), max(v[2], v[3]));
    }
    if (Bmax_) {
        uint8_t* bp = reinterpret_cast<uint8_t*>(Bmax_) + ((int64_t)row * ldb + B) * 3;
        bp[0] = (uint8_t)best;
        bp[1] = (uint8_t)(best >> 8);
        bp[2] = (uint8_t)(best >> 16);
    }
}

__global__ __launch_bounds__(256) void k_mirror_diag(float* __restrict__ M_, int64_t ldm, int32_t Ic, float* __restrict__ Bmax_, int64_t ldb) {
    mirror_diag_body(M_, ldm, Ic, Bmax_, ldb);
}
struct PanelDesc {
    float* Gp;
    float* Bmax64;
    uint32_t* Brep;
    int64_t panel_cols, ldb64;
    int32_t Ic, p_eff, nsub, pad;
};
__global__ __launch_bounds__(1024) void k_mirror_tiles_multi(const PanelDesc* __restrict__ D) {
    const PanelDesc d = D[blockIdx.z];
    if ((int)blockIdx.x >= (int)(d.panel_cols / 128) || (int)blockIdx.y >= (int)(d.panel_cols / 256) - 1) return;
    mirror_tiles_body(d.Gp, d.panel_cols, d.p_eff, nullptr, 0);
}
__global__ __launch_bounds__(256) void k_mirror_diag_multi(const PanelDesc* __restrict__ D) {
    const PanelDesc d = D[blockIdx.y];
    if ((int)blockIdx.x >= (int)(d.panel_cols / 256)) return;
    mirror_diag_body(d.Gp, d.panel_cols, d.p_eff, nullptr, 0);
}
__global__ __launch_bounds__(256) void k_panel_colmax(const PanelDesc* __restrict__ D) {
    const PanelDesc dsc = D[blockIdx.z];
    const float* __restrict__ Gp_ = dsc.Gp;
    float* __restrict__ Bmax64_ = dsc.Bmax64;
    uint32_t* __restrict__ Brep = dsc.Brep;
    const int64_t panel_cols = dsc.panel_cols, ldb64 = dsc.ldb64;
    const int32_t Ic = dsc.Ic, p_eff = dsc.p_eff, nsub = dsc.nsub;
    if ((int)blockIdx.x * 256 >= p_eff || (int)blockIdx.y * 16 >= nsub) return;
    __shared__ uint32_t sh_m[16][257], sh_r[16][257];
    const int lane = threadIdx.x & 63, wave = threadIdx.x >> 6;
    const int col0 = blockIdx.x * 256, sbg = blockIdx.y * 16;
    const int c = col0 + 4 * lane;
    const unsigned char* __restrict__ base = reinterpret_cast<const unsigned char*>(Gp_) + (int64_t)c * 3;
    const int64_t pitch = panel_cols * 3;
    for (int s = 0; s < 4; s++) {
        const int sb = sbg + 4 * wave + s;
        uint32_t t1[4] = {0, 0, 0, 0}, t2[4] = {0, 0, 0, 0};
        if (sb < nsub) {
            const int j0 = 64 * sb, nr = min(64, Ic - j0);
            for (int r = 0; r < nr; r += 8) {
                uint32_t d[8][3];
#pragma unroll
                for (int x = 0; x < 8; x++) {
                    const uint32_t* __restrict__ p = reinterpret_cast<const uint32_t*>(base + (int64_t)(j0 + min(r + x, nr - 1)) * pitch);
                    d[x][0] = p[0]; d[x][1] = p[1]; d[x][2] = p[2];
                }
#pragma unroll
                for (int x = 0; x < 8; x++) {
                    if (r + x < nr) {
                        uint32_t v[4];
                        fy_unpack24_raw(d[x][0], d[x][1], d[x][2], v);
#pragma unroll
                        for (int q = 0; q < 4; q++) {
                            const uint32_t key = (v[q] << 6) | (uint32_t)(r + x);
                            t2[q] = max(min(t1[q], key), t2[q]);
                            t1[q] = max(t1[q], key);
                        }
                    }
                }
            }
        }
#pragma unroll
        for (int q = 0; q < 4; q++) {
            sh_m[4 * wave + s][4 * lane + q] = t1[q] >> 6;
            sh_r[4 * wave + s][4 * lane + q] = (t1[q] >> 6) ? (((t2[q] >> 6) << 8) | (t1[q] & 63u)) : 0u;
        }
    }
    __syncthreads();
    const int i = col0 + threadIdx.x;
    if (i < p_eff) {
        uint32_t m[16];
#pragma unroll
        for (int k = 0; k < 16; k++) m[k] = sh_m[k][threadIdx.x];
        uint32_t* __restrict__ bp = reinterpret_cast<uint32_t*>(reinterpret_cast<unsigned char*>(Bmax64_) + ((int64_t)i * ldb64 + sbg) * 3);
#pragma unroll
        for (int g = 0; g < 4; g++) {
            const uint32_t* v = m + 4 * g;
            bp[3 * g + 0] = v[0] | (v[1] << 24);
            bp[3 * g + 1] = (v[1] >> 8) | (v[2] << 16);
            bp[3 * g + 2] = (v[2] >> 16) | (v[3] << 8);
        }
        uint32_t* __restrict__ rp = Brep + (int64_t)i * ldb64 + sbg;
#pragma unroll
        for (int k = 0; k < 16; k++) rp[k] = sh_r[k][threadIdx.x];
    }
}

static void launch_mirror(Context* ctx, float* M, int64_t ldm, int32_t Ic, float* Bmax, int64_t ldb, hipStream_t st, int bpc, const int32_t* need = nullptr,
                          int32_t write_below = 0x7FFFFFFF, bool diag = true) {
    const int nblk = (int)(ldm / 256), ntile = (int)(ldm / 128);
    const int nsrc = bpc > 0 ? nblk : nblk - 1;
    if (nblk > 1) {
        FY_HIP(hipFuncSetAttribute(reinterpret_cast<const void*>(k_mirror_tiles), hipFuncAttributeMaxDynamicSharedMemorySize, 128 * MIRROR_PITCH));
        const bool split = !need && Bmax && write_below < nsrc;
        const int ny = split ? write_below : nsrc;
        if (ny > 0) {
            k_mirror_tiles<<<dim3(ntile, ny), 1024, 128 * MIRROR_PITCH, st>>>(M, ldm, Ic, Bmax, ldb, need, write_below, bpc);
            FY_KERNEL_CHECK();
        }
        if (split) {
            k_colmax_upper<<<dim3(nblk, nsrc - write_below), 1024, 0, st>>>(M, ldm, Ic, Bmax, ldb, write_below, bpc);
            FY_KERNEL_CHECK();
        }
    }
    if (diag) {
        k_mirror_diag<<<nblk, 256, 0, st>>>(M, ldm, Ic, Bmax, ldb);
        FY_KERNEL_CHECK();
    }
}

#include "fy_rm2_kernels.hpp"
#include "fy_rm2_launch.hpp"

static_assert(TOPN_MAX == fy::TOPN_LIST_MAX, "fy_rm2.hpp states the top-N kernels' limit for the other translation units");
static void stray_allow_lds() {
    FY_HIP(hipFuncSetAttribute(reinterpret_cast<const void*>(k_score_stray), hipFuncAttributeMaxDynamicSharedMemorySize, (STRAY_UCAP + 1) * (int)sizeof(int32_t)));
}

void launch_topn_rows(Context* ctx, hipStream_t st, const float* S, int64_t ldS, int32_t n_cols, int32_t n_rows,
                      const int32_t* n_out, const int32_t* out_off, const int32_t* rank_item_raw, const int32_t* slot2du,
                      const int32_t* uid, int32_t slot0, int32_t aux_value, int32_t* out_user, int32_t* out_item,
                      float* out_score, int32_t* out_aux, int32_t* overflow, int32_t* any_overflow, int32_t top_n_hint) {
    if (n_rows <= 0) return;
    if (!st) st = ctx->stream;
    TopNArgs TA{};
    TA.S = S; TA.ldS = ldS; TA.Ic = n_cols; TA.n_out = n_out; TA.out_off = out_off; TA.rank_item_raw = rank_item_raw; TA.slot2du = slot2du; TA.uid = uid;
    TA.slot_lo = TA.slot0 = slot0;
    TA.cluster = aux_value; TA.out_user = out_user; TA.out_item = out_item; TA.out_score = out_score; TA.out_cluster = out_aux;
    launch_topn(ctx, st, TA, n_rows, overflow, any_overflow, 0, top_n_hint > TOPN_LONG, top_n_hint, nullptr);
}

}

using namespace fy;

struct TableCache {
    bool valid = false;
    std::vector<int32_t> sig;
    bool have_x = false;
    DevBuf<float> csc_x, csc_x_over_s;
    DevBuf<uint32_t> csr_pk, y_pk;
    DevBuf<int32_t> csc_rank, samples;
    CsrDescs csr_descs;
    SegStore store;
    std::vector<SegTable> segs, segs_tail;
};
struct RM2Static {
    int32_t K = 0, rank = 0, world = 1;
    int32_t max_item = -1;
    bool has_count = false;
    std::vector<int32_t> map_user, map_cluster, cluster_count;
    Smoothing smooth;
    DevBuf<double> beta_slot, s2_cluster;
    double bt_scale = 0.0;
    int32_t bt_by_n = 0;
    Prepared P;
    int32_t slot_lo = 0, slot_hi = 0;
    DevBuf<double> partial;
    bool sharded = false;
    int64_t n_raw_users = 0, n_raw_items = 0;
    std::vector<int32_t> owner;
    DevBuf<double> partial_raw;
    int deferred_code = 0;
    std::string deferred_msg;
    int64_t exchange_len() const { return sharded ? n_raw_items + 1 + n_raw_users + 1 : (int64_t)P.nI + 1; }
    DevBuf<double> b_rank, usum_slot;
    DevBuf<long long> walk_rank;
    DevBuf<int32_t> cnt_rank, deg_slot;
    DevBuf<float> fx_rank;
    std::vector<float> fx_bounds;
    double ms_build = 0;
    TableCache tables;
    std::shared_ptr<void> request_state;
    bool matches(const fy_rm2_params* prm, int64_t n_map, const int32_t* mu, const int32_t* mc, const int32_t* cc) const {
        if (K != prm->number_of_clusters || rank != prm->rank || world != prm->world || (int64_t)map_user.size() != n_map || has_count != (cc != nullptr)) return false;
        const Smoothing sm = smoothing_of(*prm);
        if (sm.method != smooth.method || (sm.general() && sm.param != smooth.param)) return false;
        if (n_map && (memcmp(map_user.data(), mu, (size_t)n_map * 4) || memcmp(map_cluster.data(), mc, (size_t)n_map * 4))) return false;
        if (cc && memcmp(cluster_count.data(), cc, (size_t)K * 4)) return false;
        return true;
    }
};

struct fy_rm2_job {
    Context* ctx = nullptr;
    fy_rm2_params prm{};
    std::shared_ptr<RM2Static> S;
    Prepared& P;
    int32_t &slot_lo, &slot_hi;
    DevBuf<double>& partial;
    DevBuf<double> stats;
    DevBuf<double> stats_raw;
    bool have_global = false;
    double ms_prepare = 0;
    bool from_cache = false;
    fy_collectives coll{};
    bool have_coll = false;
    DevBuf<double> gathered;
    DevBuf<double>&b_rank, &usum_slot;
    DevBuf<long long>& walk_rank;
    DevBuf<int32_t>&cnt_rank, &deg_slot;
    DevBuf<float>& fx_rank;
    std::vector<float>& fx_bounds;
    bool count_balanced = false;
    SmoothArgs smooth_args() const { return SmoothArgs{S->beta_slot.get(), S->deg_slot.get(), S->s2_cluster.get(), S->bt_scale, S->bt_by_n}; }
    explicit fy_rm2_job(std::shared_ptr<RM2Static> s)
        : S(std::move(s)), P(S->P), slot_lo(S->slot_lo), slot_hi(S->slot_hi), partial(S->partial), b_rank(S->b_rank), usum_slot(S->usum_slot),
          walk_rank(S->walk_rank), cnt_rank(S->cnt_rank), deg_slot(S->deg_slot), fx_rank(S->fx_rank), fx_bounds(S->fx_bounds) {}
};

static void owner_range(const fy_rm2_job* J, int k, int32_t& lo, int32_t& hi) {
    if (J->S->sharded) { lo = 0; hi = k == J->prm.rank ? J->P.nU : 0; return; }
    if (!J->count_balanced) { rank_slot_range(J->P, k, J->prm.world, lo, hi); return; }
    const int64_t n = J->P.nU, W = J->prm.world;
    lo = (int32_t)(n * k / W);
    hi = (int32_t)(n * (k + 1) / W);
}

using ScoreTune = fy::Tuning;

bool fy::gram_half_build(Context* ctx, const Prepared& P, const float* csc_w, const float* bounds3, float* G, int64_t ldm, double* ms_tables,
                         double* ms_walk, const float* csr_ones) {
    const ScoreTune tune = ctx->tune;
    const int32_t Ic = P.nP;
    if (P.K != 1 || (!csr_ones && (!P.ratings_fp16_exact || !P.ratings_positive)) || Ic <= 0) return false;
    int fxk = fx_exponent(bounds3);
    if (fxk < 0) return false;
    const int m = csr_ones ? 0 : P.ratings_frac_bits;
    const bool acc32 = tune.isim_acc32 && m <= 4 && (double)bounds3[2] * bounds3[2] * std::ldexp(1.0, 2 * m) < 16777216.0 &&
                       (double)bounds3[0] * bounds3[2] * std::ldexp(1.0, 2 * m) < 4294967296.0;
    if (acc32) fxk = 2 * m;
    int32_t CH, nch;
    pick_chunks(Ic, acc32 && !tune.cooc_max_ch_forced ? 2 * tune.cooc_max_ch : tune.cooc_max_ch, CH, nch);
    if (nch >= 256) return false;
    hipStream_t st = ctx->stream;
    cooc_rm2_allow_lds(tune.cooc_epi);
    EventTimer t_tab(ctx), t_walk(ctx);
    const size_t s0 = t_tab.begin();
    DevBuf<uint32_t> csr_pk(ctx, (size_t)P.nnz);
    DevBuf<int32_t> co(ctx, (size_t)P.nU * (nch + 1)), csc_rank(ctx, (size_t)P.nnz), samples;
    k_csc_rank<<<grid_for(P.nnz), 256, 0, st>>>(P.nnz, P.csc_pair.get(), P.pair_rank.get(), csc_rank.get());
    FY_KERNEL_CHECK();
    build_csr_samples(ctx, P.nnz, P.csr_idx.get(), samples, st);
    const CsrDescs cd = upload_csr_descs(ctx, {csr_desc(0, P.nU, CH, nch, 0, (int32_t)P.nnz)}, st);
    pack_csr(ctx, cd, P.csr_idx.get(), csr_ones ? csr_ones : P.csr_r.get(), csr_pk.get(), st);
    build_chunk_offsets(ctx, cd, P.rowptr.get(), P.csr_idx.get(), co.get(), st);
    SegStore segs;
    const SegDesc sd = seg_desc(0, 0, (int32_t)P.nnz, nch, CH, true);
    build_segment_table(ctx, SegArrays{P.csc_slot.get(), csc_w, co.get(), csc_rank.get(), samples.get()}, sd, segs, st);
    CoocArgs CA = cooc_args(P, segs.view(sd), CoocGeometry{0, 0, Ic, CH, nch, 0, (int32_t)P.nnz}, nullptr, csr_pk.get());
    CA.half = 1;
    CA.fx_scale = std::ldexp(1.0, fxk);
    CA.acc32 = acc32 ? 1 : 0;
    const int n_items = (int)cooc_item_count(Ic, CH, nch, true);
    DevBuf<int2> item_seg(ctx, (size_t)Ic * nch);
    DevBuf<int32_t> item_id(ctx, (size_t)Ic * nch), counter(ctx, 1);
    k_item_list<<<grid_for((int64_t)Ic * nch), 256, 0, st>>>(CA, item_seg.get(), item_id.get());
    FY_KERNEL_CHECK();
    CA.item_seg = item_seg.get();
    CA.item_id = item_id.get();
    counter.zero();
    CA.item_grab = cooc_item_grab(P.sum_deg2 / 2, n_items);
    MEpilogue ME{};
    ME.M = G;
    ME.ldm = ldm;
    ME.w2 = 1.0f;
    ME.fx_inv = std::ldexp(1.0, -fxk);
    t_tab.end(s0);
    const size_t s1 = t_walk.begin();
    launch_cooc_rm2(ctx, tune, true, CA, ME, n_items, counter.get(), st);
    t_walk.end(s1);
    sync(ctx);
    if (ms_tables) *ms_tables = t_tab.total_ms();
    if (ms_walk) *ms_walk = t_walk.total_ms();
    return true;
}

static_assert(PLAN_TOPN_MAX == TOPN_MAX && PLAN_TOPN_SAMPLE == TOPN_SAMPLE && PLAN_TOPN_LONG == TOPN_LONG && PLAN_SEED_CHUNKS_MAX == SEED_CHUNKS_MAX &&
                  PLAN_PRUNE_BLOCK == PRUNE_BLOCK && PLAN_STRAY_UCAP == STRAY_UCAP,
              "fy_rm2_plan.hpp and fy_rm2_kernels.hpp disagree about a limit");

struct Lane {
    hipStream_t st;
    DevBuf<float> M, S;
    DevBuf<int32_t> overflow, any_overflow;
    DevBuf<float> Bmax, amax, bmax, UB, tau;
    DevBuf<float> Gp, Bmax64, amax64, bmax64;
    DevBuf<uint32_t> Brep;
    DevBuf<uint16_t> surv;
    DevBuf<uint8_t> surv_mask;
    DevBuf<int2> strayT;
    DevBuf<int2> stray_items;
    DevBuf<int32_t> n_heavy;
    DevBuf<int32_t> need;
    DevBuf<float> Bsup, asup, bsupb, UBs;
    DevBuf<double> head32, tail32;
    DevBuf<int32_t> colmap;
    DevBuf<int32_t> sup_first;
    DevBuf<int32_t> n_quads, quad_prefix;
    DevBuf<char> scan_tmp;
    DevBuf<int2> item_seg, item_seg_t;
    DevBuf<int32_t> item_id, item_id_t;
    DevBuf<float> Ssurv;
};

struct JobArrays {
    DevBuf<double> icoll_mine;
    DevBuf<double> d_total;
    DevBuf<double> p_rank;
    DevBuf<float> a_rank, b_rank32;
    DevBuf<double2> pb_rank;
    DevBuf<float> csr_x, csr_e, csr_q;
    DevBuf<float> d_gscale;
    DevBuf<int32_t> d_cshift;
};

class SideValues {
  public:
    explicit SideValues(Context* c) : ctx(c) {}
    SideValues(const SideValues&) = delete;
    SideValues& operator=(const SideValues&) = delete;
    ~SideValues() {
        if (!joined && sv) (void)hipStreamSynchronize(sv);
        if (in) (void)hipEventDestroy(in);
        if (out) (void)hipEventDestroy(out);
    }
    void launch(hipStream_t main_stream, bool beside, const Prepared& P, double lambda, JobArrays& A, const fy_rm2_job* J) {
        if (launched) return;
        launched = true;
        hipStream_t vs = main_stream;
        if (beside && ctx->tune.overlap_values) {
            if (ctx->aux.empty()) {
                hipStream_t x;
                FY_HIP(hipStreamCreateWithFlags(&x, hipStreamNonBlocking));
                ctx->aux.push_back(x);
            }
            sv = ctx->aux[0];
            FY_HIP(hipEventCreateWithFlags(&in, hipEventDisableTiming));
            FY_HIP(hipEventCreateWithFlags(&out, hipEventDisableTiming));
            FY_HIP(hipEventRecord(in, main_stream));
            FY_HIP(hipStreamWaitEvent(sv, in, 0));
            vs = sv;
        }
        const bool general = J->S->smooth.general();
        (general ? k_csr_values<true> : k_csr_values<false>)<<<grid_for((int64_t)P.nU * 64, 256), 256, 0, vs>>>(
            P.nU, P.rowptr.get(), P.csr_idx.get(), P.csr_r.get(), P.slot2du.get(), P.ucluster.get(), P.usum.get(), P.d_csize.get(), P.d_pcstart.get(),
            A.pb_rank.get(), lambda, A.d_gscale.get(), A.csr_x.get(), A.csr_e.get(), A.csr_q.get(), general ? J->S->usum_slot.get() : nullptr,
            general ? J->smooth_args() : SmoothArgs{});
        FY_KERNEL_CHECK();
        if (vs != main_stream) {
            FY_HIP(hipEventRecord(out, sv));
            joined = false;
        }
    }
    void join(hipStream_t s) {
        if (joined) return;
        joined = true;
        FY_HIP(hipStreamWaitEvent(s, out, 0));
    }

  private:
    Context* ctx;
    hipStream_t sv = nullptr;
    hipEvent_t in = nullptr, out = nullptr;
    bool launched = false, joined = true;
};

struct ScoreShared {
    fy_rm2_job* J;
    fy_result* R;
    const ScoreTune* tune;
    const JobPlan* jp;
    const float *b_rank;
    const double *b_rank64, *p_rank;
    const float *a_rank, *csc_x, *csr_x, *csr_e, *csr_q;
    const uint32_t* csr_pk;
    const int32_t *n_out, *out_off;
    const double* pvpi;
    int32_t lo;
    const std::vector<int32_t>* csr_range;
    SideValues* side;
    EventTimer *t_cooc, *t_score, *t_topn, *t_mirror;
    unsigned long long* prune_counters;
    int64_t *blocks_total, *seed_terms_cols, *coop_survived, *fallback_survived;
    int64_t* coop_pair_contribs;
    const int32_t* cshift;
    const float* gscale;
};

static ScoreArgs score_args(const ScoreShared& X, const Plan& p, const float* M, int64_t ldm, int32_t slot0, int32_t n_users, float* S, int64_t ldS,
                            int n_slices, int n_chunks) {
    const Prepared& P = X.J->P;
    ScoreArgs SA{};
    SA.M = M; SA.ldm = ldm; SA.Ic = p.Ic; SA.a_rank = X.a_rank + p.pbase; SA.b_rank = X.b_rank + p.pbase;
    SA.rb_off = P.rowptr.get() + p.sbase;
    SA.csr_idx = P.csr_idx.get(); SA.csr_e = X.csr_e; SA.csr_q = X.csr_q;
    SA.pvpi = X.pvpi; SA.n_out = X.n_out; SA.slot_lo = X.lo; SA.slot_base = p.sbase; SA.slot0 = slot0; SA.n_users = n_users;
    SA.S = S; SA.ldS = ldS; SA.n_slices = n_slices; SA.n_chunks = n_chunks;
    return SA;
}
static void score_args_bounds(ScoreArgs& SA, int seed_chunks, const float* M2, int64_t ld2, int32_t n2, const float* a2, const float* b2, float* S2) {
    SA.chunks1 = seed_chunks;
    SA.M2 = M2; SA.ldm2 = ld2; SA.Ic2 = n2; SA.a2 = a2; SA.b2 = b2; SA.S2 = S2; SA.ldS2 = ld2; SA.no_mask2 = 1;
}
static TopNArgs topn_args(const ScoreShared& X, const Plan& p, const float* S, int64_t ldS, int32_t slot0) {
    const Prepared& P = X.J->P;
    TopNArgs TA{};
    TA.S = S; TA.ldS = ldS; TA.Ic = p.Ic; TA.n_out = X.n_out; TA.out_off = X.out_off; TA.rank_item_raw = P.rank_item_raw.get() + p.pbase;
    TA.slot2du = P.slot2du.get(); TA.uid = P.uid.get(); TA.slot_lo = X.lo; TA.slot0 = slot0; TA.cluster = p.c;
    TA.out_user = X.R->d_key0.get(); TA.out_item = X.R->d_key1.get(); TA.out_score = X.R->d_value.get(); TA.out_cluster = X.R->d_aux.get();
    return TA;
}
static void topn_pruned(TopNArgs& TA, int mode, int32_t seed_cols, const uint16_t* surv, const int32_t* n_quads, int64_t ldb, float* tau,
                        const float* Ssurv = nullptr, const int32_t* quad_prefix = nullptr) {
    TA.mode = mode; TA.seed_cols = seed_cols; TA.surv = surv; TA.n_quads = n_quads; TA.ldb = ldb; TA.tau = tau;
    TA.Ssurv = Ssurv; TA.quad_prefix = quad_prefix;
}

#include "fy_rm2_coop.hpp"

static void validate_params(const fy_rm2_params* p) {
    if (!p) FY_FAIL(FY_ERR_INVALID_ARGUMENT, "params is NULL");
    if (p->number_of_clusters <= 0) FY_FAIL(FY_ERR_INVALID_ARGUMENT, "numberOfClusters must be > 0 (got %d)", p->number_of_clusters);
    if (p->number_of_items <= 0) FY_FAIL(FY_ERR_INVALID_ARGUMENT, "numberOfItems must be > 0 (got %d)", p->number_of_items);
    const bool dir = p->flags & FY_RM2_SMOOTHING_DIRICHLET, ad = p->flags & FY_RM2_SMOOTHING_ABSOLUTE_DISCOUNT;
    if (dir && ad) FY_FAIL(FY_ERR_INVALID_ARGUMENT, "flags: FY_RM2_SMOOTHING_DIRICHLET and FY_RM2_SMOOTHING_ABSOLUTE_DISCOUNT are both set");
    if (p->flags & ~(FY_RM2_NO_CACHE | FY_RM2_SMOOTHING_DIRICHLET | FY_RM2_SMOOTHING_ABSOLUTE_DISCOUNT | FY_RM2_ESTIMATOR_RM1))
        FY_FAIL(FY_ERR_INVALID_ARGUMENT, "flags: unknown bits 0x%x", p->flags & ~15u);
    if (dir || ad) {
        if (!(std::isfinite(p->lambda) && p->lambda >= 0.0))
            FY_FAIL(FY_ERR_INVALID_ARGUMENT, "%s must be finite and >= 0 (got %g)", dir ? "mu" : "delta", p->lambda);
    } else if (!(p->lambda >= 0.0 && p->lambda <= 1.0)) FY_FAIL(FY_ERR_INVALID_ARGUMENT, "lambda must be in [0, 1]");
    if (p->world <= 0 || p->rank < 0 || p->rank >= p->world) FY_FAIL(FY_ERR_INVALID_ARGUMENT, "rank %d of world %d", p->rank, p->world);
    if (p->number_of_recommendations < 0) FY_FAIL(FY_ERR_INVALID_ARGUMENT, "numberOfRecommendations must be >= 0");
}

fy_rm2_job* fy::rm2_prepare(Context* ctx, const fy_rm2_params* prm, const fy_ratings* R, int64_t n_map, const int32_t* map_user,
// ... 519 lines not shown
                if (fd[f].empty()) continue;
                const unsigned ny = (unsigned)fd[f].size();
                F.d_flat[f].alloc(ctx, fd[f].size());
                FY_HIP(hipMemcpyAsync(F.d_flat[f].get(), fd[f].data(), fd[f].size() * sizeof(FlatDesc), hipMemcpyHostToDevice, st));
                const size_t ss = X.t_score->begin(st);
                k_count_heavy_multi<<<(ny + 63) / 64, 64, 0, st>>>(F.d_flat[f].get(), (int32_t)ny);
                FY_KERNEL_CHECK();
                score_multi_kernel(f != 0, tune.score_walk)<<<dim3((unsigned)max_grid[f], ny), 256, 0, st>>>(F.d_flat[f].get(), P.csr_idx.get(), X.csr_e, X.csr_q, X.pvpi, X.n_out);
                FY_KERNEL_CHECK();
                X.t_score->end(ss, st);
                R->st.score_launches++;
                const size_t tt = X.t_topn->begin(st);
                k_topn_fast_multi<<<dim3((unsigned)max_users[f], ny), 256, 0, st>>>(F.d_flat[f].get(), tune.force_select);
                FY_KERNEL_CHECK();
                k_topn_select_multi<<<dim3((unsigned)max_users[f], ny), 256, 0, st>>>(F.d_flat[f].get(), X.prune_counters + 2);
                FY_KERNEL_CHECK();
                X.t_topn->end(tt, st);
            }
            FY_HIP(hipStreamSynchronize(st));
        }
        first = last;
    }
}

struct PanelBuf {
    DevBuf<float> Gp, Bmax64, amax64, bmax64;
    DevBuf<uint32_t> Brep;
    DevBuf<double> head32, tail32;
};
struct PanelPtrs {
    float *Gp, *Bmax64;
    uint32_t* Brep;
    float *amax64, *bmax64;
};
struct PanelSet {
    std::vector<PanelBuf> pbuf;
    std::vector<Lane> plane;
    std::vector<CoocLaunch> batch_main, batch_tail;
    DevBuf<CoocLaunch> d_batch_main, d_batch_tail;
    DevBuf<int32_t> d_cnt_main, d_cnt_tail;
    DevBuf<PanelDesc> d_panel_desc;
    std::vector<PanelDesc> hpd;
};
static void group_buffers(Context* ctx, const JobPlan& jp, int seed_chunks, const std::vector<Lane>& lanes, int grp, PanelSet& PS) {
    const std::vector<Plan>& plans = jp.plans;
    std::vector<PanelBuf>& pbuf = PS.pbuf;
    std::vector<Lane>& plane = PS.plane;
    for (size_t pi = 0; pi < plans.size(); pi++) {
        const Plan& p = plans[pi];
        if (!p.panel || jp.group_of[pi] != grp) continue;
        pbuf[pi].Gp.alloc(ctx, (size_t)p.Ic * p.panel_cols * 3 / 4 + 4);
        pbuf[pi].Bmax64.alloc(ctx, (size_t)p.Ic * p.ldb64 * 3 / 4 + 4);
        pbuf[pi].Brep.alloc(ctx, (size_t)p.Ic * p.ldb64 + 4);
        pbuf[pi].amax64.alloc(ctx, (size_t)p.ldb64);
        pbuf[pi].bmax64.alloc(ctx, (size_t)p.ldb64);
    }
    for (size_t pi = 0; pi < plans.size(); pi++) {
        const Plan& p = plans[pi];
        if (!p.panel || jp.group_of[pi] != grp) continue;
        Lane& W = plane[pi];
        const size_t nbp = (size_t)(p.b - p.a);
        const size_t seed_cols = (size_t)std::min<int64_t>(ceil_div(p.Ic, 256), seed_chunks) * 256;
        W.st = lanes[pi % jp.NS].st;
        W.M.alloc(ctx, 1); W.Bmax.alloc(ctx, 1); W.amax.alloc(ctx, 1); W.bmax.alloc(ctx, 1);
        W.Gp.alloc(ctx, 1); W.Bmax64.alloc(ctx, 1); W.Brep.alloc(ctx, 1); W.amax64.alloc(ctx, 1); W.bmax64.alloc(ctx, 1);
        W.item_seg.alloc(ctx, (size_t)p.Ic * p.nch); W.item_id.alloc(ctx, (size_t)p.Ic * p.nch);
        W.item_seg_t.alloc(ctx, (size_t)std::max(1, p.Ic - p.p_eff)); W.item_id_t.alloc(ctx, (size_t)std::max(1, p.Ic - p.p_eff));
        W.S.alloc(ctx, nbp * seed_cols);
        W.overflow.alloc(ctx, nbp);
        W.any_overflow.alloc(ctx, 1);
        W.n_heavy.alloc(ctx, 1);
        W.UB.alloc(ctx, nbp * (size_t)p.ldb64);
        W.tau.alloc(ctx, nbp);
        W.surv.alloc(ctx, nbp * (size_t)p.ldb64);
        W.surv_mask.alloc(ctx, nbp * (size_t)p.ldb64);
        W.n_quads.alloc(ctx, nbp + 1);
        W.quad_prefix.alloc(ctx, nbp + 1);
    }
}

struct LaneGuard {
    Context* ctx;
    hipEvent_t fork = nullptr;
    int32_t* pinned = nullptr;
    ~LaneGuard() {
        for (hipStream_t x : ctx->aux) (void)hipStreamSynchronize(x);
        (void)hipStreamSynchronize(ctx->stream);
        if (fork) (void)hipEventDestroy(fork);
        if (pinned) (void)hipHostFree(pinned);
    }
};

struct ClusterVisit {
    size_t pi;
    int grp, phase;
    Lane* L;
    hipStream_t ls;
    PanelPtrs PP;
    DevBuf<double>*H32, *T32;
    Lane* own;
    PanelSet* PS;
    int32_t* pinned;
};
struct ClusterPass {
    const ScoreShared& X;
    const ClusterVisit& V;
    const Plan& p;
    Lane& L;
    hipStream_t ls;
    Context* ctx;
    const Prepared& P;
    const ScoreTune& tune;
    int fxk;
    double w2s;
    bool refine;
    int32_t head_rows;
    int64_t ld_head;
    int32_t tail_from;
    int n_chunks;
    int seed_chunks;
    bool use_sup;
    const float* Gmat;
    int64_t gld, bld, SC;
};
static ClusterPass cluster_pass(const ScoreShared& X, const ClusterVisit& V) {
    const fy_rm2_job* J = X.J;
    const ScoreTune& tune = *X.tune;
    const Plan& p = X.jp->plans[V.pi];
    ClusterPass C{X, V, p, *V.L, V.ls, J->ctx, J->P, tune};
    C.fxk = (X.jp->use_pk && tune.cooc_fx && !J->fx_bounds.empty()) ? fx_exponent(&J->fx_bounds[3 * (size_t)p.c]) : -1;
    C.w2s = J->S->smooth.w2_of(J->prm.lambda) * (double)X.gscale[(size_t)p.c];
    C.refine = tune.refine && p.pack24 && !p.coop && (C.fxk >= 0 || !tune.cooc_f32) && J->S->max_item >= 0 && J->S->max_item < (1 << 28) && p.Ic >= 8;
    C.head_rows = (int32_t)std::min<int64_t>(p.Ic & ~3, std::max<int64_t>(256, std::min<int64_t>(1024, (int64_t)tune.seed_chunks * 256)));
    C.tail_from = p.psym ? p.p_eff : p.rect ? p.CH : p.Ic;
    C.ld_head = p.psym ? (int64_t)p.p_eff : (p.rect && C.head_rows <= p.CH) ? (int64_t)p.CH : p.ldm;
    C.n_chunks = (int)ceil_div(p.Ic, 256);
    C.seed_chunks = std::min(C.n_chunks, tune.seed_chunks);
    C.use_sup = tune.sup_bounds && !p.panel && !X.jp->long_seed;
    C.Gmat = p.panel ? V.PP.Gp : V.L->M.get();
    C.gld = p.panel ? (int64_t)p.panel_cols : p.ldm;
    C.bld = p.panel ? p.ldb64 : p.ldb;
    C.SC = (int64_t)C.seed_chunks * 256;
    return C;
}
static void checkpoint(const ScoreShared& X, const ClusterVisit& V, const char* what) {
    if (X.tune->debug_sync != 1) return;
    const hipError_t e = hipDeviceSynchronize();
    fprintf(stderr, "[fy] group %d/%d phase %d plan %zu (cluster %d): %s -> %s\n", V.grp, X.jp->n_groups, V.phase, V.pi, X.jp->plans[V.pi].c, what, hipGetErrorString(e));
    fflush(stderr);
}


static void queue_row_kernel(const ScoreShared& X, const ClusterVisit& V, bool batched, bool tail, CoocArgs CA, const MEpilogue& ME, int64_t list_len,
                             int n_items, int item_grab) {
    Lane& L = *V.L;
    int2* const seg = !batched ? L.item_seg.get() : tail ? V.own->item_seg_t.get() : V.own->item_seg.get();
    int32_t* const id = !batched ? L.item_id.get() : tail ? V.own->item_id_t.get() : V.own->item_id.get();
    if (!batched) {
        k_item_list<<<grid_for(list_len), 256, 0, V.ls>>>(CA, seg, id);
        FY_KERNEL_CHECK();
    }
    CA.item_seg = seg; CA.item_id = id; CA.item_grab = item_grab;
    if (batched) {
        (tail ? V.PS->batch_tail : V.PS->batch_main).push_back(CoocLaunch{CA, ME, n_items, 0});
        return;
    }
    FY_HIP(hipMemsetAsync(L.any_overflow.get(), 0, sizeof(int32_t), V.ls));
    launch_cooc_rm2(X.J->ctx, *X.tune, X.jp->use_pk, CA, ME, n_items, L.any_overflow.get(), V.ls);
    X.R->st.cooc_launches++;
}

static void build_cluster_matrix(const ClusterPass& C) {
    const ScoreShared& X = C.X; const ClusterVisit& V = C.V; const Prepared& P = C.P; const ScoreTune& tune = C.tune; const Plan& p = C.p; Lane& L = C.L;
    Context* ctx = C.ctx;
    hipStream_t ls = C.ls;
    const TableCache& tc = X.J->S->tables;
    const JobPlan& jp = *X.jp;
    const PanelPtrs& PP = V.PP;
    const int32_t pbase = p.pbase, Ic = p.Ic;
    const int fxk = C.fxk;
    const double w2s = C.w2s;
    CoocArgs CA = cooc_args(P, tc.segs[V.pi], cooc_geometry(p), X.csr_x, X.csr_pk);
    CA.fx_scale = fxk >= 0 ? std::ldexp(1.0, fxk) : 0.0;
    MEpilogue ME{L.M.get(), p.ldm, (float)w2s, fxk >= 0 ? std::ldexp(w2s, -fxk) : 0.0,
                 p.pack24 ? 1 : 0, (p.prune && !p.panel) ? L.Bmax.get() : nullptr, p.ldb, 0,
                 p.panel ? p.panel_cols : 0, p.panel ? PP.Bmax64 : nullptr, p.ldb64, p.panel ? PP.Brep : nullptr};
    if (p.panel) ME.M = PP.Gp;
    if (C.refine) {
        V.H32->alloc(ctx, (size_t)C.head_rows * C.ld_head + 4);
        if (C.tail_from < Ic) V.T32->alloc(ctx, (size_t)std::max(1, Ic - C.tail_from) * C.head_rows + 4);
        ME.head32 = V.H32->get(); ME.ld_head = C.ld_head; ME.head_rows = C.head_rows;
        ME.tail32 = C.tail_from < Ic ? V.T32->get() : nullptr; ME.tail_from = C.tail_from;
        ME.w2d = w2s;
    }
    if (p.panel) X.R->st.panel_clusters++;
    if (p.panel || p.prune) {
        const int64_t bld = p.panel ? p.ldb64 : p.ldb;
        FY_HIP(hipMemsetAsync(p.panel ? PP.Bmax64 : L.Bmax.get(), 0, (size_t)Ic * bld * 3, ls));
        k_block_amax<<<grid_for(bld), 256, 0, ls>>>(Ic, (int32_t)bld, X.a_rank + pbase, X.b_rank + pbase, p.panel ? PP.amax64 : L.amax.get(),
                                                   p.panel ? PP.bmax64 : L.bmax.get(), p.panel ? 64 : PRUNE_BLOCK);
        FY_KERNEL_CHECK();
    }
    const size_t sp = X.t_cooc->begin(ls);
    const bool batched = V.phase == 1 && tune.panel_multi_launch && jp.use_pk && fxk >= 0 && !tune.cooc_f32;
    if (p.p_eff < Ic) {
        CoocGeometry g = cooc_geometry(p);
        g.CH = p.tail_width; g.nch = 1;
        CoocArgs CB = cooc_args(P, tc.segs_tail[V.pi], g, X.csr_x, tc.y_pk.get());
        CB.row0 = p.p_eff; CB.nrows = Ic - p.p_eff; CB.fx_scale = CA.fx_scale;
        MEpilogue MB{reinterpret_cast<float*>(reinterpret_cast<char*>(PP.Bmax64) + (size_t)(p.p_eff / 64) * 3), p.tail_width, ME.w2, ME.fx_inv, 1,
                     nullptr, 0, 0, 0, nullptr, 0, nullptr, p.ldb64, 1};
        queue_row_kernel(X, V, batched, true, CB, MB, Ic - p.p_eff, Ic - p.p_eff, 8);
        CA.tail_row0 = p.p_eff;
        CA.tail_chunks = p.tail_chunks;
    }
    CA.half = p.rect ? 2 : (p.half || p.psym) ? 1 : 0;
    if (p.psym) { CA.half_rows = p.p_eff; CA.head_chunks = p.tail_chunks; }
    const int n_items = p.psym ? (int)(cooc_half_item_index(p.p_eff - 1, p.tail_chunks - 1, p.CH, p.tail_chunks) + 1 + (int64_t)(Ic - p.p_eff) * p.tail_chunks)
                        : CA.tail_chunks > 0 ? (int)((int64_t)p.p_eff * p.nch + (int64_t)(Ic - p.p_eff) * p.tail_chunks)
                                             : (int)cooc_item_count(Ic, p.CH, p.nch, CA.half);
    const int64_t visits = (size_t)p.c < P.cluster_deg2.size() ? P.cluster_deg2[p.c] : P.sum_deg2;
    queue_row_kernel(X, V, batched, false, CA, ME, (int64_t)Ic * p.nch, n_items, cooc_item_grab(visits / (p.half ? 2 : 1), n_items));
    X.t_cooc->end(sp, ls);
    X.side->join(ls);
    checkpoint(X, V, "row kernel queued / run");
    if (p.half) {
        const size_t sm = X.t_mirror->begin(ls);
        const bool lazy = p.prune && tune.lazy_mirror;
        launch_mirror(ctx, L.M.get(), p.ldm, Ic, p.prune ? L.Bmax.get() : nullptr, p.ldb, ls, p.rect ? p.CH / 256 : 0, nullptr, lazy ? std::min(tune.seed_chunks, p.nblk) : 0x7FFFFFFF);
        X.t_mirror->end(sm, ls);
    }
    if (p.prune && !p.panel && tune.sup_bounds && !jp.long_seed) {
        std::vector<int32_t> first;
        sup_block_map(std::min(tune.seed_chunks, p.nblk), p.nblk, first);
        const int n_sup = (int)first.size() - 1;
        first.resize(65, first.back());
        L.sup_first.alloc(ctx, 65);
        L.Bsup.alloc(ctx, (size_t)Ic * 64);
        L.asup.alloc(ctx, 64); L.bsupb.alloc(ctx, 64);
        FY_HIP(hipMemcpyAsync(L.sup_first.get(), first.data(), 65 * sizeof(int32_t), hipMemcpyHostToDevice, ls));
        FY_HIP(hipStreamSynchronize(ls));
        const size_t sb = X.t_score->begin(ls);
        k_build_bsup<<<std::min<int>((Ic + 3) / 4, ctx->num_cus * 32), 256, 0, ls>>>(Ic, n_sup, L.sup_first.get(), L.Bmax.get(), p.ldb, L.Bsup.get());
        FY_KERNEL_CHECK();
        k_sup_amax<<<1, 64, 0, ls>>>(n_sup, L.sup_first.get(), L.amax.get(), L.bmax.get(), L.asup.get(), L.bsupb.get());
        FY_KERNEL_CHECK();
        X.t_score->end(sb, ls);
    }
}


struct UserBatch {
    int32_t s0, nb;
    int n_slices;
    bool whole, split;
};

static ScoreArgs batch_score_args(const ClusterPass& C, int32_t s0, int32_t nb, const float* M, int64_t ldm, float* S, int64_t ldS, int n_slices, int n_chunks) {
    ScoreArgs SA = score_args(C.X, C.p, M, ldm, s0, nb, S, ldS, n_slices, n_chunks);
    if (C.tune.score_heavy > 0) {
        const int heavy = (int64_t)nb * n_chunks < 8 * (int64_t)C.ctx->num_cus ? std::min(C.tune.score_heavy, 32) : C.tune.score_heavy;
        k_count_heavy<<<1, 64, 0, C.ls>>>(C.P.rowptr.get() + s0, nb, heavy, C.L.n_heavy.get());
        SA.n_heavy = C.L.n_heavy.get();
    }
    return SA;
}

static void refine_rows(const ClusterPass& C, int32_t s0, int32_t nb) {
    if (!C.refine || nb <= 0) return;
    const ScoreShared& X = C.X; const Prepared& P = C.P; const Plan& p = C.p; Lane& L = C.L; hipStream_t ls = C.ls;
    fy_rm2_job* J = X.J;
    const fy_rm2_params& prm = J->prm;
    const size_t tt = X.t_topn->begin(ls);
    const int32_t n_ids = J->S->max_item + 1, head_rows = C.head_rows;
    L.colmap.alloc(C.ctx, (size_t)n_ids);
    FY_HIP(hipMemsetAsync(L.colmap.get(), 0xFF, (size_t)n_ids * sizeof(int32_t), ls));
    k_refine_colmap<<<(head_rows + 255) / 256, 256, 0, ls>>>(head_rows, P.rank_item_raw.get() + p.pbase, L.colmap.get());
    FY_KERNEL_CHECK();
    RefineArgs RA{};
    RA.slot0 = s0; RA.n_users = nb; RA.slot_lo = X.lo; RA.slot_base = p.sbase;
    RA.n_out = X.n_out; RA.out_off = X.out_off; RA.out_item = X.R->d_key1.get(); RA.out_score = X.R->d_value.get(); RA.out_item_w = X.R->d_key1.get();
    RA.rowptr = P.rowptr.get(); RA.csr_idx = P.csr_idx.get(); RA.csr_r = P.csr_r.get(); RA.usum_slot = J->usum_slot.get();
    RA.p_rank = X.p_rank + p.pbase; RA.b_rank = X.b_rank64 + p.pbase;
    RA.colmap = L.colmap.get(); RA.max_item = J->S->max_item; RA.head_rows = head_rows;
    RA.head32 = C.V.H32->get(); RA.ld_head = C.ld_head; RA.tail32 = C.tail_from < p.Ic ? C.V.T32->get() : nullptr; RA.tail_from = C.tail_from;
    RA.rect_ch = p.rect ? p.CH : 0;
    if (!RA.head32 || (C.tail_from < p.Ic && !RA.tail32)) FY_FAIL(FY_ERR_STATE, "internal: cluster %d has no fp32 rows for the refinement pass", p.c);
    RA.unscale = 1.0 / (double)X.gscale[(size_t)p.c];
    RA.general = J->S->smooth.general() ? 1 : 0; RA.G = J->smooth_args(); RA.cluster = p.c;
    RA.lambda = prm.lambda; RA.ln_items = std::log((double)prm.number_of_items); RA.ln_users = std::log((double)p.Uc);
    RA.users_minus_1 = (double)(p.Uc - 1); RA.refine_c = C.tune.refine_c; RA.n_refined = X.prune_counters + 5;
    int lp2 = 64;
    while (lp2 < std::min<int>(prm.number_of_recommendations, p.Ic)) lp2 <<= 1;
    k_refine_rows<<<(nb + 3) / 4, 256, (size_t)4 * lp2 * sizeof(uint64_t), ls>>>(RA);
    FY_KERNEL_CHECK();
    X.t_topn->end(tt, ls);
}

static void batch_lists(const ClusterPass& C, int32_t s0, int32_t nb, const TopNArgs& TA, bool long_list) {
    const ScoreShared& X = C.X;
    const size_t tt = X.t_topn->begin(C.ls);
    launch_topn(C.ctx, C.ls, TA, nb, C.L.overflow.get(), C.L.any_overflow.get(), C.tune.force_select, long_list, X.J->prm.number_of_recommendations,
                X.prune_counters + 2);
    X.t_topn->end(tt, C.ls);
    refine_rows(C, s0, nb);
}

static void full_pass(const ClusterPass& C, int32_t s0, int32_t nb, float* Sx) {
    const ScoreShared& X = C.X; const Plan& p = C.p;
    const int n_slices = score_slices(C.ctx->num_cus, C.tune, nb, C.n_chunks);
    const ScoreArgs SA = batch_score_args(C, s0, nb, C.L.M.get(), p.ldm, Sx, p.ldm, n_slices, C.n_chunks);
    const size_t ss = X.t_score->begin(C.ls);
    launch_score(score_kernel(p.pack24, C.tune.score_walk), C.n_chunks * n_slices, C.ls, SA);
    X.t_score->end(ss, C.ls);
    X.R->st.score_launches++;
    batch_lists(C, s0, nb, topn_args(X, p, Sx, p.ldm, s0), X.J->prm.number_of_recommendations > TOPN_LONG);
}

static void dump_survivors(const ClusterPass& C, const UserBatch& B) {
    const Plan& p = C.p; Lane& L = C.L;
    DevBuf<int32_t> cnt(C.ctx, (size_t)p.nblk + 1);
    FY_HIP(hipMemsetAsync(cnt.get(), 0, ((size_t)p.nblk + 1) * sizeof(int32_t), C.ls));
    k_surv_block_counts<<<std::min<int>(B.nb, 4096), 64, 0, C.ls>>>(B.nb, L.n_quads.get(), L.surv.get(), p.ldb, cnt.get());
    std::vector<int32_t> hc((size_t)p.nblk + 1);
    FY_HIP(hipMemcpyAsync(hc.data(), cnt.get(), hc.size() * sizeof(int32_t), hipMemcpyDeviceToHost, C.ls));
    FY_HIP(hipStreamSynchronize(C.ls));
    int distinct = 0;
    long long total = 0;
    for (int b2 = 0; b2 < p.nblk; b2++) { distinct += hc[b2] > 0; total += hc[b2]; }
    fprintf(stderr, "[fy] cluster %d: %lld surviving (user, block) pairs in %d distinct blocks of %d:", p.c, total, distinct, p.nblk);
    for (int b2 = 0; b2 < p.nblk; b2++)
        if (hc[b2]) fprintf(stderr, " %d:%d", b2, hc[b2]);
    fprintf(stderr, "\n");
}

static void pruned_front(const ClusterPass& C, const UserBatch& B) {
    const ScoreShared& X = C.X; const Prepared& P = C.P; const ScoreTune& tune = C.tune; const Plan& p = C.p; Lane& L = C.L; hipStream_t ls = C.ls;
    Context* ctx = C.ctx;
    const PanelPtrs& PP = C.V.PP;
    const int32_t s0 = B.s0, nb = B.nb;
    const int bchunks = (int)(C.bld / 256);
    if (C.use_sup) {
        ScoreArgs SU = batch_score_args(C, s0, nb, C.Gmat, C.gld, L.S.get(), C.SC, B.n_slices, C.seed_chunks);
        L.UBs.alloc(ctx, (size_t)nb * 64);
        SU.Bsup = L.Bsup.get(); SU.asup = L.asup.get(); SU.bsup_b = L.bsupb.get(); SU.UBsup = L.UBs.get();
        SU.n_sup = std::min(64, std::max(0, p.nblk - C.seed_chunks));
        launch_score(score_sup_kernel(tune.score_walk), C.seed_chunks * B.n_slices, ls, SU);
    }
    ScoreArgs SA = batch_score_args(C, s0, nb, C.Gmat, C.gld, L.S.get(), C.SC, B.n_slices, C.seed_chunks + bchunks);
    score_args_bounds(SA, C.seed_chunks, p.panel ? PP.Bmax64 : L.Bmax.get(), C.bld, p.panel ? p.nsub : p.nblk, p.panel ? PP.amax64 : L.amax.get(),
                      p.panel ? PP.bmax64 : L.bmax.get(), L.UB.get());
    if (!C.use_sup) launch_score(score_kernel(true, tune.score_walk), (C.seed_chunks + bchunks) * B.n_slices, ls, SA);
    TopNArgs T1 = topn_args(X, p, L.S.get(), C.SC, s0);
    topn_pruned(T1, 1, C.seed_chunks * 256, L.surv.get(), L.n_quads.get(), C.bld, L.tau.get());
    if (X.jp->long_seed) {
        launch_topn_pass(ls, T1, nb, L.overflow.get(), L.any_overflow.get(), 0, true, X.J->prm.number_of_recommendations);
    } else {
        int lp2 = 64;
        while (lp2 < std::min<int>(std::min<int>(p.Ic, C.seed_chunks * 256), TOPN_SAMPLE)) lp2 <<= 1;
        topn_seed_kernel(lp2, tune.topn_seed_xl)<<<(unsigned)((nb + 3) / 4), 256, 0, ls>>>(T1, nb, L.overflow.get());
        FY_KERNEL_CHECK();
    }
    FY_HIP(hipMemsetAsync(L.n_quads.get(), 0, ((size_t)nb + 1) * sizeof(int32_t), ls));
    if (p.panel)
        k_bound_select_sub<<<grid_for((int64_t)nb * 64, 256), 256, 0, ls>>>(L.UB.get(), C.bld, p.nsub, p.nblk, C.seed_chunks, L.tau.get(),
                                                                           X.pvpi + (s0 - X.lo), nb, C.bld, L.surv.get(), L.surv_mask.get(), L.n_quads.get());
    else if (C.use_sup)
        k_bound_select_sup<<<grid_for((int64_t)nb * 64, 256), 256, 0, ls>>>(L.UBs.get(), std::min(64, std::max(0, p.nblk - C.seed_chunks)), L.sup_first.get(), L.tau.get(),
                                                                           X.pvpi + (s0 - X.lo), nb, p.ldb, L.surv.get(), L.n_quads.get());
    else
        k_bound_select<<<grid_for((int64_t)nb * 64, 256), 256, 0, ls>>>(L.UB.get(), p.ldb, p.nblk, C.seed_chunks, L.tau.get(), X.pvpi + (s0 - X.lo), nb,
                                                                       L.surv.get(), L.n_quads.get());
    FY_KERNEL_CHECK();
    if (tune.debug_sync == 3 && !p.panel) dump_survivors(C, B);
    if (p.panel && tune.panel_repair) {
        RepairArgs RA{L.surv.get(), L.surv_mask.get(), L.n_quads.get(), C.bld, nb, s0, X.lo, p.p_eff, p.Ic, P.rowptr.get(), P.csr_idx.get(),
                      X.csr_x, X.csr_e, X.csr_q, PP.Bmax64, PP.Brep, p.ldb64, PP.amax64, PP.bmax64,
                      L.tau.get(), X.pvpi, (float)C.w2s, X.prune_counters};
        k_bound_repair<<<std::min<int>(nb, ctx->num_cus * 16), 256, 0, ls>>>(RA);
        FY_KERNEL_CHECK();
    }
    if (p.half && !p.panel && tune.lazy_mirror) {
// ... 545 lines not shown
```

### filmyou-core_amd/csrc/fy_rm2_launch.hpp

```cpp
#pragma once

using ScoreKernel = void (*)(const float*, const float*, const int32_t*, const int32_t*, const float*, const float*, const double*, const int32_t*,
                             float*, ScoreArgs);
using CoocKernel = void (*)(CoocArgs, MEpilogue, int, int*);
using CoocMultiKernel = void (*)(const CoocLaunch*, int*);

static ScoreKernel score_kernel(bool pack24, int walk) {
    if (!pack24) return k_score<4, false, 8>;
    return walk ? k_score<4, true, 8, 1> : k_score<4, true, 8, 0>;
}
static auto score_multi_kernel(bool pack24, int walk) {
    if (!pack24) return k_score_multi<4, false, 8>;
    return walk ? k_score_multi<4, true, 8, 1> : k_score_multi<4, true, 8, 0>;
}
static ScoreKernel score_sup_kernel(int walk) { return walk ? k_score_sup<1> : k_score_sup<0>; }
static auto score_blocks_kernel(int walk) { return walk ? k_score_blocks<8, 1> : k_score_blocks<8, 0>; }

static auto topn_seed_kernel(int lp2, int xl) {
    static void (*const K[5][2])(TopNArgs, int32_t, int32_t*) = {{k_topn_seed<1, 0>, k_topn_seed<1, 1>}, {k_topn_seed<2, 0>, k_topn_seed<2, 1>}, {k_topn_seed<4, 0>, k_topn_seed<4, 1>},
                                                                 {k_topn_seed<8, 0>, k_topn_seed<8, 1>}, {k_topn_seed<16, 0>, k_topn_seed<16, 1>}};
    return K[lp2 <= 64 ? 0 : lp2 == 128 ? 1 : lp2 == 256 ? 2 : lp2 == 512 ? 3 : 4][xl ? 1 : 0];
}

enum CoocAcc { COOC_ACC_U64, COOC_ACC_U32, COOC_ACC_F64, COOC_ACC_F32 };
struct CoocVariant { bool pk; CoocAcc acc; int role; CoocKernel fn[2]; };
static const CoocVariant COOC_RM2_VARIANTS[] = {
    {true, COOC_ACC_U64, 0, {k_cooc_rm2<true, unsigned long long, 0, 0>, k_cooc_rm2<true, unsigned long long, 0, 1>}},
    {true, COOC_ACC_U64, 1, {k_cooc_rm2<true, unsigned long long, 1, 0>, k_cooc_rm2<true, unsigned long long, 1, 1>}},
    {true, COOC_ACC_U32, 0, {k_cooc_rm2<true, uint32_t, 0, 0>, k_cooc_rm2<true, uint32_t, 0, 1>}},
    {true, COOC_ACC_F64, 0, {k_cooc_rm2<true, double, 0, 0>, k_cooc_rm2<true, double, 0, 1>}},
    {false, COOC_ACC_F64, 0, {k_cooc_rm2<false, double, 0, 0>, k_cooc_rm2<false, double, 0, 1>}},
    {true, COOC_ACC_F32, 0, {k_cooc_rm2<true, float, 0, 0>, k_cooc_rm2<true, float, 0, 1>}},
    {false, COOC_ACC_F32, 0, {k_cooc_rm2<false, float, 0, 0>, k_cooc_rm2<false, float, 0, 1>}},
};
static const CoocMultiKernel COOC_RM2_MULTI[2][2] = {
    {k_cooc_rm2_multi<true, unsigned long long, 0, 0>, k_cooc_rm2_multi<true, unsigned long long, 0, 1>},
    {k_cooc_rm2_multi<true, unsigned long long, 1, 0>, k_cooc_rm2_multi<true, unsigned long long, 1, 1>},
};
static CoocKernel cooc_rm2_kernel(bool pk, CoocAcc acc, int role, int epi) {
    for (const CoocVariant& v : COOC_RM2_VARIANTS)
        if (v.pk == pk && v.acc == acc && v.role == role) return v.fn[epi ? 1 : 0];
    FY_FAIL(FY_ERR_STATE, "internal: no row kernel for packed %d, accumulator %d, role %d", (int)pk, (int)acc, role);
}
static CoocMultiKernel cooc_rm2_multi_kernel(int role, int epi) { return COOC_RM2_MULTI[role ? 1 : 0][epi ? 1 : 0]; }

static void cooc_rm2_allow_lds(int epi) {
    const int bytes = 160 * 1024 - 256;
    for (const CoocVariant& v : COOC_RM2_VARIANTS)
        FY_HIP(hipFuncSetAttribute(reinterpret_cast<const void*>(v.fn[epi ? 1 : 0]), hipFuncAttributeMaxDynamicSharedMemorySize, bytes));
    for (int role = 0; role < 2; role++)
        FY_HIP(hipFuncSetAttribute(reinterpret_cast<const void*>(cooc_rm2_multi_kernel(role, epi)), hipFuncAttributeMaxDynamicSharedMemorySize, bytes));
}

static void launch_score(ScoreKernel k, int grid, hipStream_t st, const ScoreArgs& A) {
    k<<<grid, 256, 0, st>>>(A.M, A.a_rank, A.rb_off, A.csr_idx, A.csr_e, A.csr_q, A.pvpi, A.n_out, A.S, A);
    FY_KERNEL_CHECK();
}

static void launch_topn_pass(hipStream_t st, const TopNArgs& TA, int32_t n_rows, int32_t* overflow, int32_t* any_overflow, int force_select, bool long_list,
                             int top_n) {
    if (long_list) k_topn_long<<<n_rows, 256, (size_t)fy_topn_long_cap(top_n) * 8, st>>>(TA, overflow, any_overflow, force_select, fy_topn_long_cap(top_n));
    else k_topn_fast<<<n_rows, 256, 0, st>>>(TA, overflow, any_overflow, force_select);
    FY_KERNEL_CHECK();
}
static void launch_topn(Context* ctx, hipStream_t st, const TopNArgs& TA, int32_t n_rows, int32_t* overflow, int32_t* any_overflow, int force_select, bool long_list,
                        int top_n, unsigned long long* n_selected) {
    FY_HIP(hipMemsetAsync(any_overflow, 0, sizeof(int32_t), st));
    launch_topn_pass(st, TA, n_rows, overflow, any_overflow, force_select, long_list, top_n);
    k_topn_select<<<fy_topn_select_grid(n_rows, ctx->num_cus), 256, 0, st>>>(TA, overflow, any_overflow, n_rows, n_selected);
    FY_KERNEL_CHECK();
}

struct CoocShape { int block, max_grid; };
static CoocShape cooc_launch_shape(size_t lds_bytes, const Tuning& tune, int num_cus) {
    const int by_lds = (int)std::max<size_t>(1, (160 * 1024 - 512) / (lds_bytes + 64));
    int block = tune.cooc_block;
    if (!block) block = by_lds >= 4 ? 256 : (by_lds >= 2 ? 512 : 1024);
    return CoocShape{block, num_cus * std::max(1, std::min(by_lds, 2048 / block))};
}
static int cooc_item_grab(int64_t visits, int64_t n_items) { return n_items > 0 && visits / n_items < 12000 ? 8 : 1; }

static void launch_cooc_rm2(Context* ctx, const Tuning& tune, bool use_pk, const CoocArgs& CA_, const MEpilogue& ME, int n_items,
                            int32_t* counter, hipStream_t st) {
    if (n_items <= 0) return;
    CoocArgs CA = CA_;
    CA.acc_quarter = tune.cooc_planes ? cooc_lds_columns(CA.CH) / 4 : 0;
    const bool fixed = use_pk && CA.fx_scale > 0.0 && !tune.cooc_f32;
    const CoocAcc acc = fixed ? (CA.acc32 ? COOC_ACC_U32 : COOC_ACC_U64) : (tune.cooc_f32 ? COOC_ACC_F32 : COOC_ACC_F64);
    const size_t lds = (size_t)cooc_lds_columns(CA.CH) * ((acc == COOC_ACC_F32 || acc == COOC_ACC_U32) ? 4 : 8);
    const CoocShape sh = cooc_launch_shape(lds, tune, ctx->num_cus);
    const int grid = std::min(n_items, sh.max_grid);
    cooc_rm2_kernel(use_pk, acc, acc == COOC_ACC_U64 && ME.ceil24 ? 1 : 0, tune.cooc_epi)<<<grid, sh.block, lds, st>>>(CA, ME, n_items, counter);
    FY_KERNEL_CHECK();
}

static void launch_cooc_rm2_multi(Context* ctx, const Tuning& tune, std::vector<CoocLaunch>& L, bool tail_role, DevBuf<CoocLaunch>& d_launch,
                                  DevBuf<int32_t>& d_counters, hipStream_t st, bool item_lists = false ) {
    if (L.empty()) return;
    int max_chp = 0, max_items = 0, max_list = 0;
    for (size_t k = 0; k < L.size(); k++)
        if (!L[k].A.item_seg || !L[k].A.item_id || !L[k].E.M || !L[k].A.seg || !L[k].A.seg_ptr || (L[k].E.panel_cols && !L[k].E.Bmax64))
            FY_FAIL(FY_ERR_STATE, "internal: launch %zu of %zu of a batched row kernel has a null operand (item_seg %p item_id %p M %p seg %p ptr %p Bmax64 %p)", k, L.size(),
                    (const void*)L[k].A.item_seg, (const void*)L[k].A.item_id, (const void*)L[k].E.M, (const void*)L[k].A.seg, (const void*)L[k].A.seg_ptr, (const void*)L[k].E.Bmax64);
    for (auto& x : L) {
        x.A.acc_quarter = tune.cooc_planes ? cooc_lds_columns(x.A.CH) / 4 : 0;
        max_chp = std::max(max_chp, cooc_lds_columns(x.A.CH));
        max_items = std::max(max_items, x.n_items);
        max_list = std::max(max_list, x.A.nrows * x.A.nch);
    }
    const size_t lds = (size_t)max_chp * 8;
    const CoocShape sh = cooc_launch_shape(lds, tune, ctx->num_cus);
    const int gx = std::max(1, std::min(max_items, sh.max_grid));
    d_launch.alloc(ctx, L.size());
    d_counters.alloc(ctx, L.size());
    FY_HIP(hipMemcpyAsync(d_launch.get(), L.data(), L.size() * sizeof(CoocLaunch), hipMemcpyHostToDevice, st));
    FY_HIP(hipMemsetAsync(d_counters.get(), 0, L.size() * sizeof(int32_t), st));
    if (item_lists) {
        k_item_list_multi<<<dim3((unsigned)std::max(1, std::min(grid_for(max_list), 4096)), (unsigned)L.size()), 256, 0, st>>>(d_launch.get());
        FY_KERNEL_CHECK();
    }
    cooc_rm2_multi_kernel(tail_role, tune.cooc_epi)<<<dim3((unsigned)gx, (unsigned)L.size()), sh.block, lds, st>>>(d_launch.get(), d_counters.get());
    FY_KERNEL_CHECK();
}
```

### filmyou-core_amd/csrc/fy_tuning.hpp

```cpp
#pragma once
#include <cstdint>

namespace fy {

struct Tuning {
    int force_select = 0;
    int pack24 = 1;
    int pack24_min_items = 4096;
    int max_slices = 65536;
    int users_per_wave = 16;
    int64_t workspace_default = (int64_t)16 << 30;
    int lanes = 4;
    bool lanes_forced = false;
    int prune = 1;
    int prune_min_items = 8192;
    int seed_chunks = 0;
    int cooc_block = 0;
    int cooc_max_ch = 19968;
    bool cooc_max_ch_forced = false;
    int sup_bounds = 1;
    int prep_packed = 1;
    int overlap_values = 1;
    int shard_prep = 1;
    int full_walk_sparse = 1;
    int refine = 1;
    float refine_c = 2.0f;
    int lazy_mirror = 1;
    int seed_forced = 0;
    int coop = 1;
    int coop_force = 0;
    int cooc_pk = 1;
    int cooc_f32 = 0;
    int cooc_half = 1;
    int cooc_rect = 1;
    int cooc_fx = 1;
    int panel_min_clusters = 4;
    int prune_min_users = 600;
    int panel_wide_below_users = 2500;
    int panel_cols = 4096;
    bool cooc_planes = true;
    int score_heavy = 512;
    int score_walk = 1;
    int cooc_epi = 1;
    int topn_seed_xl = 1;
    bool panel_repair = true;
    int panel_lanes = 2;
    int64_t flat_budget = 0;
    int64_t panel_group_bytes = 0;
    int debug_sync = 0;
    bool panel_sym = true;
    bool flat_batch = true;
    bool panel_multi_launch = true;
    bool panel_two_phase = true;
    int panel_max_ch = 4096;
    double max_surv_frac = 0.25;
    double req_full_share = 1.0;
    int req_chunk = 8192;
    int rm1_nbr_chunk = 512;
    int rm1_col_chunk = 1024;
    int upd_lds_keys = 4096;
    int isim_heavy = 4096;
    int isim_gram = -1;
    int isim_gram_min_items = 4096;
    int isim_capg = 2040;
    int isim_piece = 4096;
    int isim_acc32 = 1;
    int isim_req_chunk = 8192;
    int isim_req_rows = 0;
    int icf_est_chunk = 256;
};

inline int64_t ceil_div(int64_t a, int64_t b) { return (a + b - 1) / b; }
inline int64_t round_up(int64_t a, int64_t b) { return ceil_div(a, b) * b; }

}
```

Before: 448.7 million.

## Fuse per-run column maxima into the row kernel epilogue for rect half clusters

Adds a run-ordered item schedule for the rectangular half co-occurrence layout. Each workgroup processes groups of R consecutive rows per chunk column, keeps running per-column maxima in registers, and writes one packed partial-max row per run. The mirror and column-max pass then reads these partial rows instead of rescanning all 256 rows of each tile, which cuts memory traffic for the bounds computation. In exchange it uses extra registers, a partial-max buffer and coarser work units (one run per atomic grab), which can hurt load balance, and it applies only under narrow conditions.

```diff
diff --git a/filmyou-core_amd/_native.py b/filmyou-core_amd/_native.py
--- a/filmyou-core_amd/_native.py
+++ b/filmyou-core_amd/_native.py
@@ -8,7 +8,7 @@
 LIB_PATH = os.path.join(LIB_DIR, "libfilmyou_hip.so")
 INCLUDE = os.path.join(os.path.dirname(_HERE), "include", "filmyou.h")
 SOURCES = ["fy_api.hip", "fy_prep.hip", "fy_rm2.hip", "fy_rm2_request.hip", "fy_rm1.hip", "fy_ratings_update.hip", "fy_itemsim.hip", "fy_itemsim_request.hip", "fy_itemcf.hip", "fy_itemcf_request.hip", "fy_itemcf_estimate.hip", "fy_eval.hip", "fy_cluster.hip", "fy_nmf.hip", "fy_refine.hip", "fy_rccl.hip", "fy_seqfile.cpp"]
-HEADERS = ["fy_common.hpp", "fy_tuning.hpp", "fy_rm2_plan.hpp", "fy_rm2_tables.hpp", "fy_partition.hpp", "fy_prep.hpp", "fy_cooc.hpp", "fy_cooc_tables.hpp", "fy_rm2.hpp", "fy_rm2_kernels.hpp", "fy_rm2_launch.hpp", "fy_rm2_coop.hpp", "fy_rm2_request.hpp", "fy_rm1.hpp", "fy_ratings_update.hpp", "fy_refine.hpp", "fy_itemsim_plan.hpp", "fy_itemsim_kernels.hpp", "fy_itemsim_request.hpp", "fy_itemcf_request.hpp", "fy_eval.hpp"]
+HEADERS = ["fy_common.hpp", "fy_tuning.hpp", "fy_rm2_plan.hpp", "fy_rm2_tables.hpp", "fy_partition.hpp", "fy_prep.hpp", "fy_cooc.hpp", "fy_cooc_runs.hpp","fy_cooc_tables.hpp", "fy_rm2.hpp", "fy_rm2_kernels.hpp", "fy_rm2_launch.hpp", "fy_rm2_coop.hpp", "fy_rm2_request.hpp", "fy_rm1.hpp", "fy_ratings_update.hpp", "fy_refine.hpp", "fy_itemsim_plan.hpp", "fy_itemsim_kernels.hpp", "fy_itemsim_request.hpp", "fy_itemcf_request.hpp", "fy_eval.hpp"]
 HIPCC_FLAGS = ["--offload-arch=gfx950", "-O3", "-std=c++17", "-fPIC", "-shared", "-munsafe-fp-atomics", "-Wall",
                "-Wno-unused-result", "-ldl"]
 
diff --git a/filmyou-core_amd/csrc/fy_api.hip b/filmyou-core_amd/csrc/fy_api.hip
--- a/filmyou-core_amd/csrc/fy_api.hip
+++ b/filmyou-core_amd/csrc/fy_api.hip
@@ -56,6 +56,8 @@
     if (const char* e = getenv("FY_SCORE_HEAVY")) { int v = atoi(e); if (v >= 0) t.score_heavy = v; }
     if (const char* e = getenv("FY_SCORE_WALK")) t.score_walk = atoi(e) != 0;
     if (const char* e = getenv("FY_COOC_EPI")) t.cooc_epi = atoi(e) != 0;
+    if (const char* e = getenv("FY_COOC_RUNMAX")) t.cooc_runmax = atoi(e) != 0;
+    if (const char* e = getenv("FY_COOC_RUN_ROWS")) { int v = atoi(e); if (v == 4 || v == 8 || v == 16 || v == 32) t.cooc_run_rows = v; }
     if (const char* e = getenv("FY_TOPN_SEED_XL")) t.topn_seed_xl = atoi(e) != 0;
     if (const char* e = getenv("FY_PANEL_REPAIR")) t.panel_repair = atoi(e) != 0;
     if (const char* e = getenv("FY_PANEL_MULTI_LAUNCH")) t.panel_multi_launch = atoi(e) != 0;
diff --git a/filmyou-core_amd/csrc/fy_cooc.hpp b/filmyou-core_amd/csrc/fy_cooc.hpp
--- a/filmyou-core_amd/csrc/fy_cooc.hpp
+++ b/filmyou-core_amd/csrc/fy_cooc.hpp
@@ -4,6 +4,7 @@
 #include <type_traits>
 
 #include "fy_common.hpp"
+#include "fy_cooc_runs.hpp"
 #include "fy_prep.hpp"
 #include "fy_rm2_plan.hpp"
 #include "fy_rm2_tables.hpp"
@@ -264,7 +265,7 @@
     if (half == 2) return nrows > 0 ? cooc_rect_item_index(nrows - 1, (nrows - 1) / CH, CH) + 1 : 0;
     return nrows > 0 ? cooc_half_item_index(nrows - 1, nch - 1, CH, nch) + 1 : 0;
 }
-__device__ __forceinline__ void item_list_body(const CoocArgs& A, int2* __restrict__ seg_out, int32_t* __restrict__ id_out) {
+__device__ __forceinline__ void item_list_body(const CoocArgs& A, int2* __restrict__ seg_out, int32_t* __restrict__ id_out, const CoocRunGeom runs = CoocRunGeom{}) {
     const int n = A.nrows * A.nch;
     const int stride = A.row_stride ? A.row_stride : 1;
     for (int t = blockIdx.x * blockDim.x + threadIdx.x; t < n; t += gridDim.x * blockDim.x) {
@@ -281,7 +282,7 @@
             }
         } else if (A.half == 2) {
             if (ch > row / A.CH) continue;
-            at = cooc_rect_item_index(row, ch, A.CH);
+            at = runs.R > 0 ? cooc_run_item_index(runs, row, ch) : cooc_rect_item_index(row, ch, A.CH);
         } else if (A.half) {
             if (ch < row / A.CH) continue;
             at = cooc_half_item_index(row, ch, A.CH, A.nch);
diff --git a/filmyou-core_amd/csrc/fy_cooc_runs.hpp b/filmyou-core_amd/csrc/fy_cooc_runs.hpp
--- /dev/null
+++ b/filmyou-core_amd/csrc/fy_cooc_runs.hpp
@@ -0,0 +1,60 @@
+#pragma once
+#include <cstdint>
+
+#ifdef __HIPCC__
+#define FY_RUNS_HD __host__ __device__
+#else
+#define FY_RUNS_HD
+#endif
+
+namespace fy {
+
+constexpr int COOC_RUN_MAXTRIP = 3;
+
+struct CoocRunGeom {
+    int32_t Ic, CH;
+    int32_t R;
+    int32_t grab;
+};
+FY_RUNS_HD inline int32_t cooc_run_chunk_rows(const CoocRunGeom& g, int32_t c) { return g.Ic - c * g.CH < g.CH ? g.Ic - c * g.CH : g.CH; }
+FY_RUNS_HD inline int64_t cooc_run_item_index(const CoocRunGeom& g, int32_t row, int32_t ch) {
+    const int64_t c = row / g.CH;
+    if (c == 0) return row;
+    const int32_t rr = row - (int32_t)c * g.CH, grp = rr / g.R;
+    const int32_t left = cooc_run_chunk_rows(g, (int32_t)c) - grp * g.R, rg = left < g.R ? left : g.R;
+    return (int64_t)g.CH * (c * (c + 1) / 2) + (int64_t)grp * g.R * (c + 1) + (int64_t)ch * rg + (rr - grp * g.R);
+}
+FY_RUNS_HD inline int32_t cooc_run_head_units(const CoocRunGeom& g) { return (g.CH + g.grab - 1) / g.grab; }
+FY_RUNS_HD inline int32_t cooc_run_unit_count(const CoocRunGeom& g) {
+    int32_t n = cooc_run_head_units(g);
+    for (int32_t c = 1; c * g.CH < g.Ic; c++) n += (c + 1) * ((cooc_run_chunk_rows(g, c) + g.R - 1) / g.R);
+    return n;
+}
+FY_RUNS_HD inline void cooc_run_unit_items(const CoocRunGeom& g, int32_t u, int32_t n_items, int32_t& first, int32_t& end) {
+    const int32_t head = cooc_run_head_units(g);
+    if (u < head) {
+        first = u * g.grab;
+        end = first + g.grab < g.CH ? first + g.grab : g.CH;
+        return;
+    }
+    int32_t q = u - head;
+    for (int32_t c = 1; c * g.CH < g.Ic; c++) {
+        const int32_t rows = cooc_run_chunk_rows(g, c), runs = (c + 1) * ((rows + g.R - 1) / g.R);
+        if (q < runs) {
+            const int32_t grp = q / (c + 1), k = q - grp * (c + 1);
+            const int32_t left = rows - grp * g.R, rg = left < g.R ? left : g.R;
+            first = (int32_t)((int64_t)g.CH * ((int64_t)c * (c + 1) / 2)) + grp * g.R * (c + 1) + k * rg;
+            end = first + rg;
+            return;
+        }
+        q -= runs;
+    }
+    first = end = n_items;
+}
+FY_RUNS_HD inline bool cooc_run_same(const CoocRunGeom& g, int32_t a, int32_t b) {
+    return (a >> 8) >= g.CH && (a & 255) == (b & 255) && (a >> 8) / g.R == (b >> 8) / g.R;
+}
+FY_RUNS_HD inline int32_t cooc_run_partial_row(const CoocRunGeom& g, int32_t row) { return (row - g.CH) / g.R; }
+FY_RUNS_HD inline int32_t cooc_run_partial_rows(const CoocRunGeom& g) { return (g.Ic - g.CH + g.R - 1) / g.R; }
+
+}
diff --git a/filmyou-core_amd/csrc/fy_rm2.hip b/filmyou-core_amd/csrc/fy_rm2.hip
--- a/filmyou-core_amd/csrc/fy_rm2.hip
+++ b/filmyou-core_amd/csrc/fy_rm2.hip
@@ -446,9 +446,9 @@
         for (int k = 0; k < 4; k++) o[k] = make_double2(t[2 * k], t[2 * k + 1]);
     }
 }
-template <class ACC, bool COPY, int EPI>
+template <class ACC, bool COPY, int EPI, int RUN = 0>
 __device__ __forceinline__ void cooc_rm2_epilogue_pack(const CoocArgs& A, const MEpilogue& E, ACC* __restrict__ acc, int row, int mrow, int c0, int c1, int cb,
-                                                       int first_bmax_block) {
+                                                       int first_bmax_block, uint32_t (*rm)[8] = nullptr, bool flush = false, char* __restrict__ prow = nullptr) {
         const int64_t row_cols = E.pitch ? E.pitch : (E.panel_cols ? E.panel_cols : E.ldm);
         const uint32_t radd = E.ceil24 ? (1u << FY_P24_SHIFT) - 1u : 1u << (FY_P24_SHIFT - 1);
         if constexpr (EPI && !COPY && sizeof(ACC) == 8) {
@@ -463,7 +463,7 @@
 #pragma unroll
                 for (int q = 0; q < 4; q++) p[q] = ap[(q * qz) >> 1];
             };
-            auto trip = [&](int col, const Pair* p) __attribute__((always_inline)) {
+            auto trip = [&](int col, const Pair* p, uint32_t* rmt) __attribute__((always_inline)) {
                 const bool on = col < c1;
                 if (on) {
                     Pair* ap = reinterpret_cast<Pair*>(acc + ((col - c0) >> 2));
@@ -482,6 +482,10 @@
                         } else f = E.w2 * (float)(h ? p[q].y : p[q].x);
                         v[4 * h + q] = (__float_as_uint(f) + radd) >> FY_P24_SHIFT;
                     }
+                }
+                if constexpr (RUN) {
+#pragma unroll
+                    for (int k = 0; k < 8; k++) rmt[k] = max(rmt[k], on ? v[k] : 0u);
                 }
                 if (on) {
                     uint32_t* __restrict__ o = reinterpret_cast<uint32_t*>(out + (int64_t)col * 3);
@@ -504,14 +508,46 @@
                 }
             };
             Pair pa[4], pb[4];
+            if constexpr (RUN) {
+                static_assert(COOC_RUN_MAXTRIP == 3, "the unrolled trips below");
+                if (cw < c1) {
+                    fetch(cw + l8, pa);
+                    if (cw + step < c1) fetch(cw + step + l8, pb);
+                    trip(cw + l8, pa, rm[0]);
+                    if (cw + step < c1) {
+                        if (cw + 2 * step < c1) fetch(cw + 2 * step + l8, pa);
+                        trip(cw + step + l8, pb, rm[1]);
+                        if (cw + 2 * step < c1) trip(cw + 2 * step + l8, pa, rm[2]);
+                    }
+                }
+                if (flush) {
+#pragma unroll
+                    for (int t = 0; t < COOC_RUN_MAXTRIP; t++) {
+                        const int col = cw + t * step + l8;
+                        uint32_t* const v = rm[t];
+                        if (col < c1) {
+                            uint32_t* __restrict__ o = reinterpret_cast<uint32_t*>(prow + (int64_t)col * 3);
+                            o[0] = v[0] | (v[1] << 24);
+                            o[1] = (v[1] >> 8) | (v[2] << 16);
+                            o[2] = (v[2] >> 16) | (v[3] << 8);
+                            o[3] = v[4] | (v[5] << 24);
+                            o[4] = (v[5] >> 8) | (v[6] << 16);
+                            o[5] = (v[6] >> 16) | (v[7] << 8);
+                        }
+#pragma unroll
+                        for (int k = 0; k < 8; k++) v[k] = 0u;
+                    }
+                }
+                return;
+            }
             if (cw < c1) fetch(cw + l8, pa);
             while (cw < c1) {
                 if (cw + step < c1) fetch(cw + step + l8, pb);
-                trip(cw + l8, pa);
+                trip(cw + l8, pa, nullptr);
                 cw += step;
                 if (cw >= c1) break;
                 if (cw + step < c1) fetch(cw + step + l8, pa);
-                trip(cw + l8, pb);
+                trip(cw + l8, pb, nullptr);
                 cw += step;
             }
             return;
@@ -588,8 +624,13 @@
         }
 }
 
-template <class ACC, int EPI>
-__device__ __forceinline__ void cooc_rm2_epilogue(const CoocArgs& A, const MEpilogue& E, ACC* __restrict__ acc, int id) {
+struct CoocRunArgs {
+    CoocRunGeom g;
+    unsigned char* __restrict__ Pm;
+};
+template <class ACC, int EPI, int RUN = 0>
+__device__ __forceinline__ void cooc_rm2_epilogue(const CoocArgs& A, const MEpilogue& E, ACC* __restrict__ acc, int id, uint32_t (*rm)[8] = nullptr, bool flush = false,
+                                                  const CoocRunArgs* Rn = nullptr) {
     const int lrow = id >> 8;
     const int row = A.row0 + lrow * (A.row_stride ? A.row_stride : 1);
     const int mrow = E.local_rows ? lrow : row;
@@ -606,6 +647,13 @@
         if (copy) cooc_rm2_epilogue_pack<ACC, true, EPI>(A, E, acc, row, mrow, c0, c1, cb, first_bmax_block);
         else {
             if (tail8) cooc_rm2_tail_copy<ACC>(A, E, acc, row, c0, min(c1, (int)E.head_rows));
+            if constexpr (RUN) {
+                if (row >= A.CH) {
+                    char* prow = reinterpret_cast<char*>(Rn->Pm) + (int64_t)cooc_run_partial_row(Rn->g, row) * E.ldm * 3;
+                    cooc_rm2_epilogue_pack<ACC, false, EPI, 1>(A, E, acc, row, mrow, c0, c1, cb, first_bmax_block, rm, flush, prow);
+                    return;
+                }
+            }
             cooc_rm2_epilogue_pack<ACC, false, EPI>(A, E, acc, row, mrow, c0, c1, cb, first_bmax_block);
         }
     } else {
@@ -619,8 +667,8 @@
     }
 }
 
-template <bool PK, class ACC, int EPI>
-__device__ __forceinline__ void cooc_rm2_body(const CoocArgs& A, const MEpilogue& E, int n_items, int* __restrict__ next_item) {
+template <bool PK, class ACC, int EPI, int RUN = 0>
+__device__ __forceinline__ void cooc_rm2_body(const CoocArgs& A, const MEpilogue& E, int n_items, int* __restrict__ next_item, const CoocRunArgs* Rn = nullptr) {
     ACC* __restrict__ acc = reinterpret_cast<ACC*>(fy_cooc_acc);
     __shared__ int sh_item, sh_s0, sh_s1, sh_id;
     const int CHp = cooc_lds_columns(A.CH);
@@ -628,18 +676,32 @@
     const int ITEM_GRAB = A.item_grab > 0 ? A.item_grab : 1;
     int next = 0, next2 = 0;
     int g_cur = 0, g_end = 0, g_next = 0;
+    uint32_t rm[RUN ? COOC_RUN_MAXTRIP : 1][8] = {};
     auto grab = [&]() __attribute__((always_inline)) {
         if (g_cur == g_end) {
+            if constexpr (RUN) {
+                cooc_run_unit_items(Rn->g, g_next, n_items, g_cur, g_end);
+                if (g_cur >= n_items) g_end = g_cur + 1;
+                g_next = atomicAdd(next_item, 1);
+            } else {
             g_cur = g_next;
             g_end = g_cur + ITEM_GRAB;
             g_next = atomicAdd(next_item, ITEM_GRAB);
+            }
         }
         return g_cur++;
     };
     if (threadIdx.x == 0) {
+        if constexpr (RUN) {
+            const int u = atomicAdd(next_item, 1);
+            g_next = atomicAdd(next_item, 1);
+            cooc_run_unit_items(Rn->g, u, n_items, g_cur, g_end);
+            if (g_cur >= n_items) g_end = g_cur + 1;
+        } else {
         g_cur = atomicAdd(next_item, ITEM_GRAB);
         g_end = g_cur + ITEM_GRAB;
         g_next = atomicAdd(next_item, ITEM_GRAB);
+        }
         const int first = grab();
         next = grab();
         const int2 se = first < n_items ? A.item_seg[first] : make_int2(0, 0);
@@ -671,7 +733,8 @@
         s1 = sh_s1;
         const int nid = sh_id;
         batch = cooc_first_batch(A, s0, s1);
-        cooc_rm2_epilogue<ACC, EPI>(A, E, acc, id);
+        if constexpr (RUN) cooc_rm2_epilogue<ACC, EPI, 1>(A, E, acc, id, rm, !(nitem < n_items && cooc_run_same(Rn->g, id, nid)), Rn);
+        else cooc_rm2_epilogue<ACC, EPI>(A, E, acc, id);
         item = nitem;
         id = nid;
         if (threadIdx.x == 0) next = next2;
@@ -681,6 +744,13 @@
 template <bool PK, class ACC, int ROLE = 0, int EPI = 1>
 __global__ void k_cooc_rm2(CoocArgs A, MEpilogue E, int n_items, int* __restrict__ next_item) {
     cooc_rm2_body<PK, ACC, EPI>(A, E, n_items, next_item);
+}
+template <bool PK, class ACC>
+__global__ void k_cooc_rm2_runs(CoocArgs A, MEpilogue E, int n_items, int* __restrict__ next_item, CoocRunArgs Rn) {
+    cooc_rm2_body<PK, ACC, 1, 1>(A, E, n_items, next_item, &Rn);
+}
+__global__ void k_item_list_runs(CoocArgs A, int2* __restrict__ seg_out, int32_t* __restrict__ id_out, CoocRunGeom runs) {
+    item_list_body(A, seg_out, id_out, runs);
 }
 struct CoocLaunch {
     CoocArgs A;
@@ -775,8 +845,9 @@
                                                        const int32_t* __restrict__ need, int32_t write_below, int32_t bpc) {
     mirror_tiles_body(M_, ldm, Ic, Bmax_, ldb, need, write_below, bpc);
 }
-__global__ __launch_bounds__(1024) void k_colmax_upper(const float* __restrict__ M_, int64_t ldm, int32_t Ic, float* __restrict__ Bmax_, int64_t ldb, int32_t first_block,
-                                                       int32_t bpc) {
+template <bool RUNS>
+__device__ __forceinline__ void colmax_upper_body(const float* __restrict__ M_, int64_t ldm, int32_t Ic, float* __restrict__ Bmax_, int64_t ldb, int32_t first_block,
+                                                  int32_t bpc, int32_t run_rows = 0, int32_t run_from = 0) {
     __shared__ uint32_t colmax[256];
     const int tj = blockIdx.x, B = first_block + blockIdx.y;
     if (tj == B || !cooc_tile_stored(B, tj, bpc) || 256 * B >= Ic) return;
@@ -789,6 +860,18 @@
     __syncthreads();
     uint32_t mx[4] = {0, 0, 0, 0};
     const int r_end = min(256, Ic - 256 * B);
+    if constexpr (RUNS) {
+        const int n_src = (r_end + run_rows - 1) / run_rows;
+        const int64_t src0 = (256 * B - run_from) / run_rows;
+#pragma unroll 4
+        for (int r = wave; r < n_src; r += (int)(blockDim.x >> 6)) {
+            const uint32_t* __restrict__ p = reinterpret_cast<const uint32_t*>(Mb + (src0 + r) * pitch + (int64_t)col0 * 3) + 3 * lane;
+            uint32_t v[4];
+            fy_unpack24_raw(p[0], p[1], p[2], v);
+#pragma unroll
+            for (int q = 0; q < 4; q++) mx[q] = max(mx[q], v[q]);
+        }
+    } else {
     uint32_t d[4][3];
 #pragma unroll
     for (int step = 0; step < 4; step++) {
@@ -805,6 +888,7 @@
 #pragma unroll
             for (int q = 0; q < 4; q++) mx[q] = max(mx[q], v[q]);
         }
+    }
     }
 #pragma unroll
     for (int q = 0; q < 4; q++)
@@ -817,6 +901,14 @@
         bp[1] = (uint8_t)(pv >> 8);
         bp[2] = (uint8_t)(pv >> 16);
     }
+}
+__global__ __launch_bounds__(1024) void k_colmax_upper(const float* __restrict__ M_, int64_t ldm, int32_t Ic, float* __restrict__ Bmax_, int64_t ldb, int32_t first_block,
+                                                       int32_t bpc) {
+    colmax_upper_body<false>(M_, ldm, Ic, Bmax_, ldb, first_block, bpc);
+}
+__global__ __launch_bounds__(1024) void k_colmax_runs(const float* __restrict__ Pm_, int64_t ldm, int32_t Ic, float* __restrict__ Bmax_, int64_t ldb, int32_t first_block,
+                                                      int32_t bpc, int32_t run_rows, int32_t run_from) {
+    colmax_upper_body<true>(Pm_, ldm, Ic, Bmax_, ldb, first_block, bpc, run_rows, run_from);
 }
 __global__ void k_flag_surviving_blocks(int32_t n_users, const int32_t* __restrict__ n_quads, const uint16_t* __restrict__ surv, int64_t ldb, int32_t* __restrict__ need) {
     for (int32_t u = blockIdx.x; u < n_users; u += gridDim.x)
@@ -946,7 +1038,7 @@
 }
 
 static void launch_mirror(Context* ctx, float* M, int64_t ldm, int32_t Ic, float* Bmax, int64_t ldb, hipStream_t st, int bpc, const int32_t* need = nullptr,
-                          int32_t write_below = 0x7FFFFFFF, bool diag = true) {
+                          int32_t write_below = 0x7FFFFFFF, bool diag = true, const unsigned char* Pm = nullptr, int32_t run_rows = 0, int32_t run_from = 0) {
     const int nblk = (int)(ldm / 256), ntile = (int)(ldm / 128);
     const int nsrc = bpc > 0 ? nblk : nblk - 1;
     if (nblk > 1) {
@@ -957,8 +1049,13 @@
             k_mirror_tiles<<<dim3(ntile, ny), 1024, 128 * MIRROR_PITCH, st>>>(M, ldm, Ic, Bmax, ldb, need, write_below, bpc);
             FY_KERNEL_CHECK();
         }
-        if (split) {
-            k_colmax_upper<<<dim3(nblk, nsrc - write_below), 1024, 0, st>>>(M, ldm, Ic, Bmax, ldb, write_below, bpc);
+        const int runs_first = split && Pm && run_rows > 0 ? std::min(nsrc, std::max<int>(write_below, run_from / 256)) : nsrc;
+        if (split && runs_first > write_below) {
+            k_colmax_upper<<<dim3(nblk, runs_first - write_below), 1024, 0, st>>>(M, ldm, Ic, Bmax, ldb, write_below, bpc);
+            FY_KERNEL_CHECK();
+        }
+        if (split && runs_first < nsrc) {
+            k_colmax_runs<<<dim3(nblk, nsrc - runs_first), 256, 0, st>>>(reinterpret_cast<const float*>(Pm), ldm, Ic, Bmax, ldb, runs_first, bpc, run_rows, run_from);
             FY_KERNEL_CHECK();
         }
     }
@@ -1142,6 +1239,7 @@
 struct Lane {
     hipStream_t st;
     DevBuf<float> M, S;
+    DevBuf<unsigned char> Pm;
     DevBuf<int32_t> overflow, any_overflow;
     DevBuf<float> Bmax, amax, bmax, UB, tau;
     DevBuf<float> Gp, Bmax64, amax64, bmax64;
@@ -1967,12 +2065,13 @@
 
 
 static void queue_row_kernel(const ScoreShared& X, const ClusterVisit& V, bool batched, bool tail, CoocArgs CA, const MEpilogue& ME, int64_t list_len,
-                             int n_items, int item_grab) {
+                             int n_items, int item_grab, const CoocRunArgs* Rn = nullptr) {
     Lane& L = *V.L;
     int2* const seg = !batched ? L.item_seg.get() : tail ? V.own->item_seg_t.get() : V.own->item_seg.get();
     int32_t* const id = !batched ? L.item_id.get() : tail ? V.own->item_id_t.get() : V.own->item_id.get();
     if (!batched) {
-        k_item_list<<<grid_for(list_len), 256, 0, V.ls>>>(CA, seg, id);
+        if (Rn) k_item_list_runs<<<grid_for(list_len), 256, 0, V.ls>>>(CA, seg, id, Rn->g);
+        else k_item_list<<<grid_for(list_len), 256, 0, V.ls>>>(CA, seg, id);
         FY_KERNEL_CHECK();
     }
     CA.item_seg = seg; CA.item_id = id; CA.item_grab = item_grab;
@@ -1981,7 +2080,7 @@
         return;
     }
     FY_HIP(hipMemsetAsync(L.any_overflow.get(), 0, sizeof(int32_t), V.ls));
-    launch_cooc_rm2(X.J->ctx, *X.tune, X.jp->use_pk, CA, ME, n_items, L.any_overflow.get(), V.ls);
+    launch_cooc_rm2(X.J->ctx, *X.tune, X.jp->use_pk, CA, ME, n_items, L.any_overflow.get(), V.ls, Rn);
     X.R->st.cooc_launches++;
 }
 
@@ -2035,14 +2134,28 @@
                         : CA.tail_chunks > 0 ? (int)((int64_t)p.p_eff * p.nch + (int64_t)(Ic - p.p_eff) * p.tail_chunks)
                                              : (int)cooc_item_count(Ic, p.CH, p.nch, CA.half);
     const int64_t visits = (size_t)p.c < P.cluster_deg2.size() ? P.cluster_deg2[p.c] : P.sum_deg2;
-    queue_row_kernel(X, V, batched, false, CA, ME, (int64_t)Ic * p.nch, n_items, cooc_item_grab(visits / (p.half ? 2 : 1), n_items));
+    const int item_grab = cooc_item_grab(visits / (p.half ? 2 : 1), n_items);
+    const bool eight = p.pack24 && !p.panel && tune.cooc_epi && tune.cooc_planes && !tune.cooc_f32;
+    const int run_rows = cooc_run_rows(tune.cooc_runmax, tune.cooc_run_rows, CA.half, p.half && p.prune && tune.lazy_mirror && ME.Bmax, batched, eight, p.CH,
+                                       cooc_rm2_block(tune, p.CH, ctx->num_cus), C.refine ? C.head_rows : 0);
+    CoocRunArgs RA{CoocRunGeom{Ic, p.CH, run_rows, item_grab}, nullptr};
+    if (run_rows > 0) {
+        L.Pm.alloc(ctx, (size_t)cooc_run_partial_rows(RA.g) * p.ldm * 3);
+        RA.Pm = L.Pm.get();
+        for (int32_t r0 = p.CH; r0 < Ic; r0 += run_rows) {
+            const int64_t c = r0 / p.CH, c1 = c == p.nch - 1 ? p.ldm : (c + 1) * p.CH;
+            X.R->st.cooc_matrix_bytes += 3 * (c * p.CH + c1 - (r0 & ~255));
+        }
+    }
+    queue_row_kernel(X, V, batched, false, CA, ME, (int64_t)Ic * p.nch, n_items, item_grab, run_rows > 0 ? &RA : nullptr);
     X.t_cooc->end(sp, ls);
     X.side->join(ls);
     checkpoint(X, V, "row kernel queued / run");
     if (p.half) {
         const size_t sm = X.t_mirror->begin(ls);
         const bool lazy = p.prune && tune.lazy_mirror;
-        launch_mirror(ctx, L.M.get(), p.ldm, Ic, p.prune ? L.Bmax.get() : nullptr, p.ldb, ls, p.rect ? p.CH / 256 : 0, nullptr, lazy ? std::min(tune.seed_chunks, p.nblk) : 0x7FFFFFFF);
+        launch_mirror(ctx, L.M.get(), p.ldm, Ic, p.prune ? L.Bmax.get() : nullptr, p.ldb, ls, p.rect ? p.CH / 256 : 0, nullptr, lazy ? std::min(tune.seed_chunks, p.nblk) : 0x7FFFFFFF,
+                      true, run_rows > 0 ? L.Pm.get() : nullptr, run_rows, p.CH);
         X.t_mirror->end(sm, ls);
     }
     if (p.prune && !p.panel && tune.sup_bounds && !jp.long_seed) {
diff --git a/filmyou-core_amd/csrc/fy_rm2_launch.hpp b/filmyou-core_amd/csrc/fy_rm2_launch.hpp
--- a/filmyou-core_amd/csrc/fy_rm2_launch.hpp
+++ b/filmyou-core_amd/csrc/fy_rm2_launch.hpp
@@ -4,6 +4,7 @@
                              float*, ScoreArgs);
 using CoocKernel = void (*)(CoocArgs, MEpilogue, int, int*);
 using CoocMultiKernel = void (*)(const CoocLaunch*, int*);
+using CoocRunsKernel = void (*)(CoocArgs, MEpilogue, int, int*, CoocRunArgs);
 
 static ScoreKernel score_kernel(bool pack24, int walk) {
     if (!pack24) return k_score<4, false, 8>;
@@ -37,6 +38,17 @@
     {k_cooc_rm2_multi<true, unsigned long long, 0, 0>, k_cooc_rm2_multi<true, unsigned long long, 0, 1>},
     {k_cooc_rm2_multi<true, unsigned long long, 1, 0>, k_cooc_rm2_multi<true, unsigned long long, 1, 1>},
 };
+struct CoocRunsVariant { bool pk; CoocAcc acc; CoocRunsKernel fn; };
+static const CoocRunsVariant COOC_RM2_RUNS[] = {
+    {true, COOC_ACC_U64, k_cooc_rm2_runs<true, unsigned long long>},
+    {true, COOC_ACC_F64, k_cooc_rm2_runs<true, double>},
+    {false, COOC_ACC_F64, k_cooc_rm2_runs<false, double>},
+};
+static CoocRunsKernel cooc_rm2_runs_kernel(bool pk, CoocAcc acc) {
+    for (const CoocRunsVariant& v : COOC_RM2_RUNS)
+        if (v.pk == pk && v.acc == acc) return v.fn;
+    FY_FAIL(FY_ERR_STATE, "internal: no row kernel with runs for packed %d, accumulator %d", (int)pk, (int)acc);
+}
 static CoocKernel cooc_rm2_kernel(bool pk, CoocAcc acc, int role, int epi) {
     for (const CoocVariant& v : COOC_RM2_VARIANTS)
         if (v.pk == pk && v.acc == acc && v.role == role) return v.fn[epi ? 1 : 0];
@@ -50,6 +62,8 @@
         FY_HIP(hipFuncSetAttribute(reinterpret_cast<const void*>(v.fn[epi ? 1 : 0]), hipFuncAttributeMaxDynamicSharedMemorySize, bytes));
     for (int role = 0; role < 2; role++)
         FY_HIP(hipFuncSetAttribute(reinterpret_cast<const void*>(cooc_rm2_multi_kernel(role, epi)), hipFuncAttributeMaxDynamicSharedMemorySize, bytes));
+    if (epi)
+        for (const CoocRunsVariant& v : COOC_RM2_RUNS) FY_HIP(hipFuncSetAttribute(reinterpret_cast<const void*>(v.fn), hipFuncAttributeMaxDynamicSharedMemorySize, bytes));
 }
 
 static void launch_score(ScoreKernel k, int grid, hipStream_t st, const ScoreArgs& A) {
@@ -80,8 +94,16 @@
 }
 static int cooc_item_grab(int64_t visits, int64_t n_items) { return n_items > 0 && visits / n_items < 12000 ? 8 : 1; }
 
+static int cooc_run_rows(int runmax, int run_rows, int half, bool lazy_bounds, bool batched, bool eight, int CH, int block, int copy_rows) {
+    if (!runmax || half != 2 || !lazy_bounds || batched || !eight || block <= 0 || CH % 256 != 0 || copy_rows > CH) return 0;
+    if (run_rows != 4 && run_rows != 8 && run_rows != 16 && run_rows != 32) return 0;
+    const int trips = (cooc_lds_columns(CH) + 8 * block - 1) / (8 * block);
+    return trips <= COOC_RUN_MAXTRIP ? run_rows : 0;
+}
+static int cooc_rm2_block(const Tuning& tune, int CH, int num_cus) { return cooc_launch_shape((size_t)cooc_lds_columns(CH) * 8, tune, num_cus).block; }
+
 static void launch_cooc_rm2(Context* ctx, const Tuning& tune, bool use_pk, const CoocArgs& CA_, const MEpilogue& ME, int n_items,
-                            int32_t* counter, hipStream_t st) {
+                            int32_t* counter, hipStream_t st, const CoocRunArgs* Rn = nullptr) {
     if (n_items <= 0) return;
     CoocArgs CA = CA_;
     CA.acc_quarter = tune.cooc_planes ? cooc_lds_columns(CA.CH) / 4 : 0;
@@ -89,6 +111,15 @@
     const CoocAcc acc = fixed ? (CA.acc32 ? COOC_ACC_U32 : COOC_ACC_U64) : (tune.cooc_f32 ? COOC_ACC_F32 : COOC_ACC_F64);
     const size_t lds = (size_t)cooc_lds_columns(CA.CH) * ((acc == COOC_ACC_F32 || acc == COOC_ACC_U32) ? 4 : 8);
     const CoocShape sh = cooc_launch_shape(lds, tune, ctx->num_cus);
+    if (Rn && Rn->g.R > 0) {
+        if ((acc != COOC_ACC_U64 && acc != COOC_ACC_F64) || !tune.cooc_epi || !CA.acc_quarter || ME.ceil24 ||
+            (cooc_lds_columns(CA.CH) + 8 * sh.block - 1) / (8 * sh.block) > COOC_RUN_MAXTRIP)
+            FY_FAIL(FY_ERR_STATE, "internal: a row kernel with runs for accumulator %d, epilogue %d, planes %d, workgroup %d", (int)acc, tune.cooc_epi, CA.acc_quarter, sh.block);
+        const int grid = std::min(cooc_run_unit_count(Rn->g), sh.max_grid);
+        cooc_rm2_runs_kernel(use_pk, acc)<<<grid, sh.block, lds, st>>>(CA, ME, n_items, counter, *Rn);
+        FY_KERNEL_CHECK();
+        return;
+    }
     const int grid = std::min(n_items, sh.max_grid);
     cooc_rm2_kernel(use_pk, acc, acc == COOC_ACC_U64 && ME.ceil24 ? 1 : 0, tune.cooc_epi)<<<grid, sh.block, lds, st>>>(CA, ME, n_items, counter);
     FY_KERNEL_CHECK();
diff --git a/filmyou-core_amd/csrc/fy_tuning.hpp b/filmyou-core_amd/csrc/fy_tuning.hpp
--- a/filmyou-core_amd/csrc/fy_tuning.hpp
+++ b/filmyou-core_amd/csrc/fy_tuning.hpp
@@ -42,6 +42,8 @@
     int score_heavy = 512;
     int score_walk = 1;
     int cooc_epi = 1;
+    int cooc_runmax = 1;
+    int cooc_run_rows = 16;
     int topn_seed_xl = 1;
     bool panel_repair = true;
     int panel_lanes = 2;
```

Result: faster. 453.6 million, median of 6 (+1.1%).
